# nikisalli/nightmare_rl

Measured on AMD Instinct MI355X. Metric: env-steps/sec at N parallel Nightmare-v3 envs, 1/2/4/8 MI355X, higher is better.
Workload: dtype f32; 1 GPU; 4096 Nightmare-v3 envs per GPU, random-action rollout U(-1,1)^18, full step(): 2 x 8 ms substeps (18-DoF dynamics + floor contact, PGS x3 + noslip x4) + obs/reward/termination/reset; envs_per_gpu=4096, decimation=2

## Files before the change

include/nightmare_hip.h:

```cpp
#ifndef NIGHTMARE_HIP_H
#define NIGHTMARE_HIP_H
#include <stdint.h>
#ifdef __cplusplus
extern "C" {
#endif

#define NM_NUM_OBS 66
#define NM_NUM_ACTIONS 18
#define NM_NUM_REWARDS 16
#define NM_DTYPE_F32 0
#define NM_DTYPE_F64 1

typedef struct nm_env nm_env;

typedef struct {
  int32_t decimation;
  double p_gain;
  double action_scale;
  double default_pos[3];
  double clip_actions;
  double clip_observations;
  double obs_lin_vel, obs_ang_vel, obs_dof_pos, obs_dof_vel;
  double episode_length_s;
  double resampling_time;
// ... 43 lines not shown

int nm_set_observation_noise(nm_env* env, const double* noise_scale_vec_host);
int nm_set_noise_uniforms(nm_env* env, const double* u_host);
int nm_set_push(nm_env* env, int32_t interval_steps, double max_vel_xy, uint64_t start_step);
int nm_get_push(nm_env* env, int32_t* interval_steps, double* max_vel_xy, uint64_t* step);
int nm_set_reset_noise(nm_env* env, const double* ranges10_host, const uint32_t* counts_host);
int nm_get_reset_noise(nm_env* env, int32_t* on, double* ranges10, uint32_t* counts_host);
int nm_reset_noise_offsets(const double* ranges10, uint64_t seed, int64_t global_env, uint32_t k, int32_t dtype, double* out43);
int nm_set_env_params(nm_env* env, const void* mu_dev, const void* p_gain_dev, const void* kv_dev, void* stream);
int nm_get_env_params(nm_env* env, void* mu_dev, void* p_gain_dev, void* kv_dev, void* stream);
int nm_draw_env_params(nm_env* env, const double lo[3], const double hi[3], void* stream);
int nm_set_body_params(nm_env* env, const void* rows_dev, void* stream);
int nm_get_body_params(nm_env* env, void* out_dev, void* stream);
int nm_draw_payload(nm_env* env, const double lo[4], const double hi[4], void* out_dev, void* stream);
int nm_set_action_latency(nm_env* env, const int32_t* substeps_dev, void* stream);
int nm_get_action_latency(nm_env* env, int32_t* out_dev, void* stream);
int nm_draw_action_latency(nm_env* env, int32_t lo, int32_t hi, void* stream);
int nm_set_action_history(nm_env* env, const float* hist_dev, void* stream);
int nm_get_action_history(nm_env* env, float* out_dev, void* stream);
int nm_set_gravity(nm_env* env, const void* rows_dev, void* stream);
int nm_get_gravity(nm_env* env, void* out_dev, void* stream);
int nm_draw_gravity(nm_env* env, const double lo[5], const double hi[5], void* out_dev, void* stream);
int nm_set_servo(nm_env* env, const void* rows_dev, void* stream);
int nm_get_servo(nm_env* env, void* out_dev, void* stream);
int nm_draw_servo(nm_env* env, const double lo[2], const double hi[2], void* stream);
int nm_get_servo_state(nm_env* env, double* limited);
int nm_set_servo_state(nm_env* env, const double* limited);
int nm_set_state_record(nm_env* env, int32_t env_index);
int nm_get_state_record(nm_env* env, double* qpos, double* qvel, int32_t* bad_state_resets);
int nm_get_state_log(nm_env* env, int32_t first_step, int32_t count, double* rows_host);
int nm_get_state_log_dones(nm_env* env, int32_t first_step, int32_t count, unsigned char* dones_host);

int nm_profile(nm_env* env, int32_t enable, double* sum_ms, int64_t* count);

typedef enum {
  NM_ACT_ELU = 0,
  NM_ACT_SELU = 1,
  NM_ACT_RELU = 2,
  NM_ACT_LRELU = 3,
  NM_ACT_TANH = 4,
  NM_ACT_SIGMOID = 5
} nm_activation;
#define NM_NUM_ACTIVATIONS 6

typedef struct nm_policy nm_policy;
int nm_policy_create(const int32_t* dims, int32_t n_layers, int32_t device, nm_policy** out);
int nm_policy_create_act(const int32_t* dims, int32_t n_layers, int32_t activation, int32_t device, nm_policy** out);
int nm_policy_destroy(nm_policy* h);
int nm_policy_load(nm_policy* h, const float* const* weights_dev, const float* const* bias_dev, void* stream);
int nm_policy_forward(nm_policy* h, const float* obs_dev, int32_t num_envs, float* out_dev, void* stream);

int nm_gae(const float* rewards_dev, const float* values_dev, const unsigned char* dones_dev, const float* last_values_dev,
           int32_t T, int32_t N, float gamma, float lam, float* returns_dev, void* stream);
int nm_gae_advantages(const float* rewards_dev, const float* values_dev, const unsigned char* dones_dev, const float* last_values_dev, int32_t T, int32_t N,
                      float gamma, float lam, float* returns_dev, float* advantages_dev, float* scratch_dev, int32_t normalize, void* stream);

int nm_ppo_sample(const float* net_out_dev, const float* std_dev, const float* obs_dev, int32_t N, int32_t A, int32_t n_obs, uint64_t seed,
                  const int64_t* iter_dev, int32_t step, float* actions_dev, float* logp_dev, float* values_dev, float* mu_dev, float* sigma_dev,
                  float* obs_store_dev, void* stream);
int nm_ppo_record(const float* rew_dev, const int64_t* done_dev, const float* time_outs_dev, const float* values_dev, float gamma, int32_t N,
                  float* rewards_store_dev, unsigned char* dones_store_dev, float* cur_ret_dev, float* cur_len_dev, float* fin3_dev,
                  const float* ep_stats_dev, const int32_t* ep_idx_dev, int32_t n_ep, float* ep_acc_dev, void* stream);

typedef struct nm_ppo nm_ppo;
int nm_ppo_create(const int32_t* actor_dims, const int32_t* critic_dims, int32_t n_layers, int32_t device, nm_ppo** out);
int nm_ppo_create_act(const int32_t* actor_dims, const int32_t* critic_dims, int32_t n_layers, int32_t activation, int32_t device, nm_ppo** out);
// ... 121 lines not shown
```

nightmare_rl_amd/_lib.py:

```python
import ctypes as C
import os

HERE = os.path.dirname(os.path.abspath(__file__))
LIB_PATH = os.environ.get("NM_HIP_LIB") or os.path.join(HERE, "csrc", "libnightmare_hip.so")
NUM_OBS, NUM_ACTIONS, NUM_REWARDS = 66, 18, 16
DTYPE_F32, DTYPE_F64 = 0, 1
ACTIVATIONS = {"elu": 0, "selu": 1, "relu": 2, "crelu": 2, "lrelu": 3, "tanh": 4, "sigmoid": 5}


def activation_code(name):
    try:
        return ACTIVATIONS[name]
    except (KeyError, TypeError):
        raise ValueError(f"activation {name!r} has no kernel (known: {sorted(ACTIVATIONS)})") from None


EXPORTS = ["nm_default_config", "nm_reward_name", "nm_last_error", "nm_create", "nm_destroy", "nm_num_envs", "nm_dtype", "nm_reset",
           "nm_step", "nm_step_physics", "nm_get_state", "nm_set_state", "nm_get_buffers", "nm_set_buffers",
           "nm_set_command_uniforms", "nm_get_feet_state", "nm_set_feet_state", "nm_get_counters", "nm_set_debug_buffer", "nm_set_return_accumulator", "nm_invalidate_time_outs", "nm_rollout", "nm_rollout_act", "nm_rollout_supported", "nm_policy_create", "nm_policy_destroy", "nm_policy_load", "nm_policy_forward", "nm_profile", "nm_gae", "nm_gae_advantages", "nm_ppo_sample", "nm_ppo_record", "nm_ppo_create", "nm_ppo_destroy", "nm_ppo_num_params", "nm_ppo_sync_params", "nm_ppo_minibatch", "nm_ppo_minibatch_rows", "nm_ppo_set_storage_rows", "nm_ppo_step_is_fused", "nm_ppo_debug_break_barrier", "nm_ppo_permutation", "nm_ppo_copy_grad", "nm_ppo_set_grad_buffer", "nm_ppo_get_state", "nm_ppo_snapshot_state", "nm_ppo_has_fast_path", "nm_ppo_act", "nm_ppo_record_act",
           "nm_policy_create_act", "nm_ppo_create_act", "nm_rollout_supported_act", "nm_rollout_ex", "nm_rollout_act_ex",
           "nm_set_observation_noise", "nm_set_noise_uniforms", "nm_set_state_record", "nm_get_state_record",
           "nm_get_state_log", "nm_get_state_log_dones", "nm_play", "nm_play_supported",
           "nm_nik_create", "nm_nik_destroy", "nm_nik_reset", "nm_nik_set_gait", "nm_nik_update", "nm_nik_get_state",
           "nm_step_tape", "nm_nik_tape", "nm_set_push", "nm_get_push",
           "nm_set_env_params", "nm_get_env_params", "nm_draw_env_params",
           "nm_set_body_params", "nm_get_body_params", "nm_draw_payload",
           "nm_set_action_latency", "nm_get_action_latency", "nm_draw_action_latency", "nm_set_action_history", "nm_get_action_history",
           "nm_set_reset_noise", "nm_get_reset_noise", "nm_reset_noise_offsets",
           "nm_set_gravity", "nm_get_gravity", "nm_draw_gravity",
           "nm_set_servo", "nm_get_servo", "nm_draw_servo", "nm_get_servo_state", "nm_set_servo_state"]


class NmConfig(C.Structure):
    _fields_ = [("decimation", C.c_int32), ("p_gain", C.c_double), ("action_scale", C.c_double), ("default_pos", C.c_double * 3),
                ("clip_actions", C.c_double), ("clip_observations", C.c_double),
                ("obs_lin_vel", C.c_double), ("obs_ang_vel", C.c_double), ("obs_dof_pos", C.c_double), ("obs_dof_vel", C.c_double),
                ("episode_length_s", C.c_double), ("resampling_time", C.c_double), ("max_lin_vel_x", C.c_double), ("max_ang_vel", C.c_double),
                ("termination_contact_force", C.c_double), ("tracking_sigma", C.c_double), ("reward_scales", C.c_double * NUM_REWARDS),
                ("tibia_contact_mode", C.c_int32), ("tibia_max_contact_force", C.c_double), ("body_contact_mode", C.c_int32),
                ("body_max_contact_force", C.c_double), ("base_height_target", C.c_double), ("max_contact_force", C.c_double)]


class NmRolloutArgs(C.Structure):
    _fields_ = [("steps", C.c_int32), ("params_flat_dev", C.c_void_p), ("seed", C.c_uint64), ("iter_dev", C.c_void_p),
                ("obs0_dev", C.c_void_p), ("obs_final_dev", C.c_void_p), ("episode_length_dev", C.c_void_p),
                ("rew_dev", C.c_void_p), ("done_dev", C.c_void_p), ("time_outs_dev", C.c_void_p), ("ep_stats_dev", C.c_void_p), ("bootstrap_time_outs", C.c_int32),
                ("s_obs", C.c_void_p), ("s_actions", C.c_void_p), ("s_logp", C.c_void_p), ("s_values", C.c_void_p), ("s_mu", C.c_void_p),
                ("s_sigma", C.c_void_p), ("s_rewards", C.c_void_p), ("s_dones", C.c_void_p), ("gamma", C.c_float),
                ("cur_ret", C.c_void_p), ("cur_len", C.c_void_p), ("fin3", C.c_void_p),
                ("ep_idx_dev", C.c_void_p), ("n_ep", C.c_int32), ("ep_acc_dev", C.c_void_p), ("last_values_dev", C.c_void_p)]


class NmPlayArgs(C.Structure):
    _fields_ = [("steps", C.c_int32), ("deterministic", C.c_int32), ("params_flat_dev", C.c_void_p), ("seed", C.c_uint64), ("iter_dev", C.c_void_p),
                ("step0", C.c_uint64), ("obs0_dev", C.c_void_p), ("obs_dev", C.c_void_p), ("actions_dev", C.c_void_p), ("episode_length_dev", C.c_void_p),
                ("rew_dev", C.c_void_p), ("done_dev", C.c_void_p), ("time_outs_dev", C.c_void_p), ("ep_stats_dev", C.c_void_p),
                ("cur_ret", C.c_void_p), ("cur_len", C.c_void_p), ("fin3", C.c_void_p), ("ret_sum", C.c_void_p), ("ret_cnt", C.c_void_p),
                ("ep_idx_dev", C.c_void_p), ("n_ep", C.c_int32), ("ep_acc_dev", C.c_void_p)]


class NmTapeArgs(C.Structure):
    _fields_ = [("steps", C.c_int32), ("actions_dev", C.c_void_p), ("obs_dev", C.c_void_p), ("episode_length_dev", C.c_void_p),
                ("rew_dev", C.c_void_p), ("done_dev", C.c_void_p), ("time_outs_dev", C.c_void_p), ("ep_stats_dev", C.c_void_p),
# ... 94 lines not shown
    if hasattr(L, "nm_step_tape"):
        L.nm_step_tape.argtypes = [vp, C.POINTER(NmTapeArgs), vp]
    if hasattr(L, "nm_set_push"):
        L.nm_set_push.argtypes = [vp, C.c_int32, C.c_double, C.c_uint64]
        L.nm_get_push.argtypes = [vp, C.POINTER(C.c_int32), C.POINTER(C.c_double), C.POINTER(C.c_uint64)]
    if hasattr(L, "nm_set_env_params"):
        L.nm_set_env_params.argtypes = [vp, vp, vp, vp, vp]
        L.nm_get_env_params.argtypes = [vp, vp, vp, vp, vp]
        L.nm_draw_env_params.argtypes = [vp, C.POINTER(C.c_double * 3), C.POINTER(C.c_double * 3), vp]
    if hasattr(L, "nm_set_body_params"):
        L.nm_set_body_params.argtypes = [vp, vp, vp]
        L.nm_get_body_params.argtypes = [vp, vp, vp]
        L.nm_draw_payload.argtypes = [vp, C.POINTER(C.c_double * 4), C.POINTER(C.c_double * 4), vp, vp]
    if hasattr(L, "nm_set_action_latency"):
        L.nm_set_action_latency.argtypes = [vp, vp, vp]
        L.nm_get_action_latency.argtypes = [vp, vp, vp]
        L.nm_draw_action_latency.argtypes = [vp, C.c_int32, C.c_int32, vp]
        L.nm_set_action_history.argtypes = [vp, vp, vp]
        L.nm_get_action_history.argtypes = [vp, vp, vp]
    if hasattr(L, "nm_set_reset_noise"):
        L.nm_set_reset_noise.argtypes = [vp, C.POINTER(C.c_double * 10), vp]
        L.nm_get_reset_noise.argtypes = [vp, C.POINTER(C.c_int32), C.POINTER(C.c_double * 10), vp]
        L.nm_reset_noise_offsets.argtypes = [C.POINTER(C.c_double * 10), C.c_uint64, C.c_int64, C.c_uint32, C.c_int32, C.POINTER(C.c_double * 43)]
    if hasattr(L, "nm_set_gravity"):
        L.nm_set_gravity.argtypes = [vp, vp, vp]
        L.nm_get_gravity.argtypes = [vp, vp, vp]
        L.nm_draw_gravity.argtypes = [vp, C.POINTER(C.c_double * 5), C.POINTER(C.c_double * 5), vp, vp]
    if hasattr(L, "nm_set_servo"):
        L.nm_set_servo.argtypes = [vp, vp, vp]
        L.nm_get_servo.argtypes = [vp, vp, vp]
        L.nm_draw_servo.argtypes = [vp, C.POINTER(C.c_double * 2), C.POINTER(C.c_double * 2), vp]
        L.nm_get_servo_state.argtypes = [vp, vp]
        L.nm_set_servo_state.argtypes = [vp, vp]
    if not full:
        return L
    L.nm_gae.argtypes = [vp, vp, vp, vp, C.c_int32, C.c_int32, C.c_float, C.c_float, vp, vp]
    L.nm_gae_advantages.argtypes = [vp, vp, vp, vp, C.c_int32, C.c_int32, C.c_float, C.c_float, vp, vp, vp, C.c_int32, vp]
    L.nm_ppo_sample.argtypes = [vp, vp, vp, C.c_int32, C.c_int32, C.c_int32, C.c_uint64, vp, C.c_int32, vp, vp, vp, vp, vp, vp, vp]
    L.nm_ppo_record.argtypes = [vp, vp, vp, vp, C.c_float, C.c_int32, vp, vp, vp, vp, vp, vp, vp, C.c_int32, vp, vp]
    L.nm_ppo_create.argtypes = [vp, vp, C.c_int32, C.c_int32, C.POINTER(vp)]
    L.nm_ppo_create_act.argtypes = [vp, vp, C.c_int32, C.c_int32, C.c_int32, C.POINTER(vp)]
    L.nm_ppo_destroy.argtypes = [vp]
    L.nm_ppo_num_params.argtypes = [vp]
    L.nm_ppo_sync_params.argtypes = [vp, vp, C.c_float, C.c_int64, vp]
    L.nm_ppo_minibatch.argtypes = [vp] * 12 + [C.c_int32, C.c_int32, C.c_float, C.c_float, C.c_float, C.c_int32, C.c_float, C.c_int32, C.c_float,
                                               C.c_float, C.c_float, C.c_float, C.c_int32, C.c_float, vp]
    L.nm_ppo_minibatch_rows.argtypes = [vp] * 13 + [C.c_int32, C.c_int32, C.c_float, C.c_float, C.c_float, C.c_int32, C.c_float, C.c_int32, C.c_float,
                                                    C.c_float, C.c_float, C.c_float, C.c_int32, C.c_float, vp]
    L.nm_ppo_permutation.argtypes = [vp, C.c_int32, C.c_uint64, C.c_uint64, vp]
    L.nm_ppo_copy_grad.argtypes = [vp, vp, C.c_int32, vp]
    L.nm_ppo_set_grad_buffer.argtypes = [vp, vp]
    L.nm_ppo_has_fast_path.argtypes = [vp]
    L.nm_ppo_act.argtypes = [vp, vp, vp, C.c_int32, C.c_uint64, vp, C.c_int32, vp, vp, vp, vp, vp, vp, vp]
    L.nm_ppo_record_act.argtypes = [vp, vp, vp, vp, vp, C.c_float, vp, vp, vp, vp, vp, vp, vp, C.c_int32, vp,
                                    vp, vp, C.c_int32, C.c_uint64, vp, C.c_int32, vp, vp, vp, vp, vp, vp, vp]
    L.nm_ppo_get_state.argtypes = [vp, vp, C.c_int32, vp]
    L.nm_ppo_set_storage_rows.argtypes = [vp, C.c_int64]
    L.nm_ppo_step_is_fused.argtypes = [vp]
    L.nm_ppo_step_is_fused.restype = C.c_int32
    L.nm_ppo_debug_break_barrier.argtypes = [vp, vp]
    L.nm_ppo_snapshot_state.argtypes = [vp, vp, C.c_int32, vp]
    L.nm_policy_create.argtypes = [vp, C.c_int32, C.c_int32, C.POINTER(vp)]
    L.nm_policy_create_act.argtypes = [vp, C.c_int32, C.c_int32, C.c_int32, C.POINTER(vp)]
    L.nm_policy_destroy.argtypes = [vp]
    L.nm_policy_load.argtypes = [vp, vp, vp, vp]
    L.nm_policy_forward.argtypes = [vp, vp, C.c_int32, vp, vp]
# ... 21 lines not shown
```

nightmare_rl_amd/csrc/nm_core.h:

```cpp
#pragma once
#include <type_traits>
#include <stddef.h>

#include "simt.h"

#ifdef NM_MEASURE
#define NM_ABLATE(mask) (mask)
#else
#define NM_ABLATE(mask) 0
#endif
namespace nm {
using namespace simt;

constexpr int kNQ = 25, kNV = 24, kNU = 18, kNLEG = 6, kNCOL = 7, kNSENS = 13, kNOBS = 66, kNREW = 16;
constexpr int kLinkN = 25;
constexpr int kLegN = 3 * kLinkN;
constexpr int kBaseN = 10;
constexpr int kColN = 24;
constexpr int kMaxCon = 16;
constexpr int kMaxRow = 4 * kMaxCon;
constexpr int kMaxConBig = 44;
constexpr int kBigSlots = (4 * kMaxConBig + NM_WAVE - 1) / NM_WAVE;
constexpr int kJRow = 16;
enum { R_ACTION_RATE, R_ANG_VEL_XY, R_BASE_HEIGHT, R_BODY_CONTACT, R_DEFAULT_POS, R_DOF_ACC, R_DOF_VEL, R_FEET_AIR_TIME, R_FEET_CONTACT,
// ... 96 lines not shown
  const VR d = Tt - Lo;
  return sel(vabs(d) <= rate, Tt, sel(d < VR(0), Lo - rate, Lo + rate));
}
constexpr int kDbgN = 256;

template <class Src> struct ArgSrc { static constexpr bool kScalarBase = false; };
template <class real> NM_FN const Args<real>& launch_args(const Args<real>& a) { return a; }
template <class real> NM_FN const Args<real>& launch_args(const Args<real>* a) { return *a; }
#ifndef NM_EMUL
typedef const __attribute__((address_space(4))) char* kernarg_ptr;
template <class real, int OFS> struct KernArgs { kernarg_ptr seg; };
template <class real, int OFS> struct ArgSrc<KernArgs<real, OFS>> { static constexpr bool kScalarBase = true; };
template <class real, int OFS> NM_FN const Args<real>& launch_args(const KernArgs<real, OFS>& k) {
  kernarg_ptr p = k.seg;
  asm volatile("" : "+s"(p));
  return *(const Args<real>*)(const __attribute__((address_space(4))) Args<real>*)(p + OFS);
}
template <class real, int OFS> NM_FN void launch_args_touch(const KernArgs<real, OFS>& k) {
  kernarg_ptr p = k.seg;
  asm volatile("" : "+s"(p));
  int x = 0;
#pragma unroll
  for (int o = 0; o < OFS + (int)sizeof(Args<real>); o += 64) x |= *(const __attribute__((address_space(4))) int*)(p + o);
  asm volatile("" ::"s"(x));
}
template <class real> NM_FN const Args<real>* scalar_src(const Args<real>* a) { return a; }
template <class real, int OFS> NM_FN KernArgs<real, OFS> scalar_src(const KernArgs<real, OFS>& k) {
  const uint64_t u = (uint64_t)k.seg;
  const uint32_t lo = (uint32_t)__builtin_amdgcn_readfirstlane((int)(uint32_t)u), hi = (uint32_t)__builtin_amdgcn_readfirstlane((int)(uint32_t)(u >> 32));
  return KernArgs<real, OFS>{(kernarg_ptr)(((uint64_t)hi << 32) | lo)};
}
#endif

template <class real> struct Sh {
  real qpos[kNQ];
  real envp[kEnvPS];
  real qvel[24], warm[24], ctrl[20];
  real Rb[9], wv[6];
  real anc[kNU * 3], axs[kNU * 3];
  real colR[kNCOL * 9], colp[kNCOL * 3];
  real Minv[kNLEG * 6], W[kNLEG * 18], Lb[15], Dbi[6];
  real MinvH[kNLEG * 6], WH[kNLEG * 18], LbH[15], DbiH[6];
  real qas[24], qfs[24], qfc[24];
  real vv[24];
  real sens[16], cvb[6];
  real bh[2];
  real mbb[36], sc[36];
  real legtmp[kNLEG * 66];
  NM_FN real* cpos() { return legtmp; }
  NM_FN real* cnrm() { return legtmp + 3 * kMaxConBig; }
  NM_FN real* cdist() { return legtmp + 6 * kMaxConBig; }
  NM_FN int* cleg() { return reinterpret_cast<int*>(legtmp + 7 * kMaxConBig); }
  NM_FN int* cleg1() { return reinterpret_cast<int*>(legtmp + 8 * kMaxConBig); }
  real efc_f[kMaxRow];
#ifdef NM_DEBUG_SOLVER
  real dbg_b[kMaxRow], dbg_a[kMaxRow], dbg_f0[kMaxRow];
#endif
  int ncon, nwarn, it_pgs, it_noslip, anypair;
  int nhop;
  int ntog;
  real eact[kNU], epact[kNU], epdv[kNU];
  real ecmd[4], eepsum[kNREW];
  int eplen_lo, eplen_hi;
  unsigned ectr;
  int cstart[8], ccnt[8];
  real sink[NM_WAVE];
// ... 212 lines not shown

#if defined(NM_STAMPS) && !defined(NM_EMUL)
__device__ unsigned long long g_stamps[16];
NM_FN void nm_stamp(int k) {
  __shared__ unsigned long long tl, acc[16];
#ifdef NM_STAMPS_B
  asm volatile("s_waitcnt vmcnt(0) lgkmcnt(0)" ::: "memory");
#endif
  unsigned long long n = __builtin_amdgcn_s_memtime();
  if (NM_TID == 0) {
    if (k < 0) for (int i = 0; i < 16; i++) acc[i] = 0;
    else acc[k] += n - tl;
    if (k == 10) for (int i = 0; i < 16; i++) atomicAdd(&g_stamps[i], acc[i]);
    tl = n;
  }
}
#else
NM_FN void nm_stamp(int) {}
#endif
#ifdef NM_STAMPS_B
#define NM_ESTAMP(k)
#define NM_BSTAMP(k) nm_stamp(k)
#else
#define NM_ESTAMP(k) nm_stamp(k)
#define NM_BSTAMP(k)
#endif

constexpr int kLinkTmp = 22;

template <class real> NM_FN V<real> legsum(const V<real>& x, const VB& isleg) {
  return gsum8(sel(isleg, x, V<real>(real(0))));
}

template <int EP, class real, int G> NM_FN void stage_smooth(ShW<real, G>& w, const Model<real>& M, bool last) {
  typedef V<real> vr;
  real* lds = reinterpret_cast<real*>(&w.e[0]);
  static_assert((G & (G - 1)) == 0 && 2 * G <= 8, "lane groups: G envs x 2 factorisations");
  const V<int> lane0 = opaque_lane();
  const V<int> sub = lane0 & 7, grp = lane0 >> 3;
  const V<int> leg = vmin(sub, V<int>(5)), eo = (grp & (G - 1)) * (int)(sizeof(Sh<real>) / sizeof(real));
  const VB pass1 = (grp & G) != 0;
  const VB isleg = sub < V<int>(6);
#define LDG(field, i) ldsv(lds, eo + (NM_OFS(field) + (i)))
  const V<int> bo = (grp & (G - 1)) * kBodyP + (int)(sizeof(ShW<real, G>) / sizeof(real));
#define LDB(i) ldsv(lds, bo + (i))
  const VB st_all = VB(true), st_leg = VB(true);
#define STG(field, i, val) stsv(lds, eo + (NM_OFS(field) + (i)), val, st_all)
#define LDL(field, idx) ldsv(lds, eo + (idx) + NM_OFS(field))
#define STL(field, idx, val) stsv(lds, eo + (idx) + NM_OFS(field), val, st_leg)
  const V<int> slot = leg * (3 * kLinkTmp);

  vr Rb[9];
  {
    vr qw = LDG(qpos, 3), qx = LDG(qpos, 4), qy = LDG(qpos, 5), qz = LDG(qpos, 6);
    {
      const vr in_ = vrcp(vsqrt(qw * qw + qx * qx + qy * qy + qz * qz));
      qw = qw * in_; qx = qx * in_; qy = qy * in_; qz = qz * in_;
      STG(qpos, 3, qw); STG(qpos, 4, qx); STG(qpos, 5, qy); STG(qpos, 6, qz);
    }
    vr q00 = qw * qw, q01 = qw * qx, q02 = qw * qy, q03 = qw * qz, q11 = qx * qx, q12 = qx * qy, q13 = qx * qz, q22 = qy * qy,
       q23 = qy * qz, q33 = qz * qz;
    Rb[0] = q00 + q11 - q22 - q33; Rb[4] = q00 - q11 + q22 - q33; Rb[8] = q00 - q11 - q22 + q33;
    Rb[1] = real(2) * (q12 - q03); Rb[2] = real(2) * (q13 + q02); Rb[3] = real(2) * (q12 + q03);
    Rb[5] = real(2) * (q23 - q01); Rb[6] = real(2) * (q13 - q02); Rb[7] = real(2) * (q23 + q01);
  }
  vr vb[6], ab[6];
  {
// ... 31 lines not shown
    vr Rl[9];
    Rl[0] = co + oc * ax[0] * ax[0]; Rl[1] = oc * ax[0] * ax[1] - s_ * ax[2]; Rl[2] = oc * ax[0] * ax[2] + s_ * ax[1];
    Rl[3] = oc * ax[0] * ax[1] + s_ * ax[2]; Rl[4] = co + oc * ax[1] * ax[1]; Rl[5] = oc * ax[1] * ax[2] - s_ * ax[0];
    Rl[6] = oc * ax[0] * ax[2] - s_ * ax[1]; Rl[7] = oc * ax[1] * ax[2] + s_ * ax[0]; Rl[8] = co + oc * ax[2] * ax[2];
#pragma unroll
    for (int j = 0; j < 9; j++) STL(legtmp, leg * 27 + lk * 9 + j, Rl[j]);
    wave_sync();
  }
#endif
  vr mcom[3] = {vr(real(0)), vr(real(0)), vr(real(0))};
  {
    vr Rp[9], pp[3], vpar[6], apar[6];
    vr cR[9], cpos[3], cS[6], cv[6], ca[6];
#pragma unroll
    for (int k = 0; k < 9; k++) Rp[k] = Rb[k];
    pp[0] = pp[1] = pp[2] = vr(real(0));
#pragma unroll
    for (int k = 0; k < 6; k++) { vpar[k] = vb[k]; apar[k] = ab[k]; }
#pragma unroll
    for (int k = 0; k < 3; k++) {
      sched_fence();
      const V<int> cb = leg * kLegN + k * kLinkN;
      vr q = LDL(qpos, leg * 3 + (7 + k)), qd = LDL(qvel, leg * 3 + (6 + k));
      vr pos[3], t3[3], aw[3], R[9];
      {
        vr bpos[3] = {ldsv(M.legc, cb), ldsv(M.legc, cb + 1), ldsv(M.legc, cb + 2)};
        matvec3(t3, Rp, bpos);
        pos[0] = pp[0] + t3[0]; pos[1] = pp[1] + t3[1]; pos[2] = pp[2] + t3[2];
      }
      {
        vr ax[3] = {ldsv(M.legc, cb + 12), ldsv(M.legc, cb + 13), ldsv(M.legc, cb + 14)};
        vr R0[9];
        {
          if (uniform(M.link_rot_id[k])) {
#pragma unroll
            for (int j = 0; j < 9; j++) R0[j] = Rp[j];
          } else {
            vr bR[9];
#pragma unroll
            for (int j = 0; j < 9; j++) bR[j] = ldsv(M.legc, cb + 3 + j);
            matmul3(R0, Rp, bR);
          }
        }
        matvec3(aw, R0, ax);
        vr Rl[9];
#ifndef NM_NO_ROLE_ROT
#pragma unroll
        for (int j = 0; j < 9; j++) Rl[j] = LDL(legtmp, leg * 27 + (k * 9 + j));
        (void)q;
#else
        vr s, co;
        vsincos(q, &s, &co);
        vr oc = vr(real(1)) - co;
        Rl[0] = co + oc * ax[0] * ax[0]; Rl[1] = oc * ax[0] * ax[1] - s * ax[2]; Rl[2] = oc * ax[0] * ax[2] + s * ax[1];
        Rl[3] = oc * ax[0] * ax[1] + s * ax[2]; Rl[4] = co + oc * ax[1] * ax[1]; Rl[5] = oc * ax[1] * ax[2] - s * ax[0];
        Rl[6] = oc * ax[0] * ax[2] - s * ax[1]; Rl[7] = oc * ax[1] * ax[2] + s * ax[0]; Rl[8] = co + oc * ax[2] * ax[2];
#endif
        matmul3(R, R0, Rl);
      }
#pragma unroll
      for (int j = 0; j < 3; j++) {
        STL(anc, leg * 9 + (3 * k + j), pos[j]);
        STL(axs, leg * 9 + (3 * k + j), aw[j]);
      }
      if (k == 2) {
#pragma unroll
        for (int j = 0; j < 9; j++) STL(colR, (leg + 1) * 9 + j, R[j]);
// ... 619 lines not shown
  wmaxfirst(best, &sv, &si);
  if (popc64(ballot(best == vr(sv))) == 1) return rdlane(ibest, si);
  wargmax(best, ibest, &sv, &si);
  return si;
}
template <class real> NM_FN real hull_tie_tol() { return sizeof(real) == 8 ? real(1e-13) : real(4e-7); }
constexpr int kMaxHop = 3;
template <class real> constexpr real kObbSlack() { return real(1e-5); }

constexpr int kSelfLane = 63;
constexpr int kSlackScale = 1 << 20;
constexpr int kBatchLane0 = kSelfLane + 1 - kNCOL;
template <class real> NM_FN void hull_ring(const Model<real>& M, int gv, V<int>& nbg, V<real>* v) {
  const V<int> lane = lane_id();
  const VB nbl = lane < M.maxnbr;
  V<real> o[4];
  gld4(M.hullnv, (sel(nbl, lane, V<int>(M.maxnbr)) + gv * (M.maxnbr + 1)) * 4, o);
  v[0] = o[0]; v[1] = o[1]; v[2] = o[2];
  nbg = to_int(o[3]);
}
template <class real> struct Rings {
  V<int> nb[kNCOL];
  V<real> vv[kNCOL][3];
  int cur[kNCOL];
};
template <class real> NM_FN void collide_rings(const Sh<real>& sh, const Model<real>& M, Rings<real>& r) {
#pragma unroll
  for (int g = 0; g < kNCOL; g++) {
    const int vadr = (int)M.colc[kColN * g + 6];
    r.cur[g] = uniform(sh.hcache[g]);
    hull_ring(M, vadr + r.cur[g], r.nb[g], r.vv[g]);
  }
}
template <class real> NM_FN void stage_collide(Sh<real>& sh, const Model<real>& M, int* dropped, Rings<real>& rg, bool pairs = true) {
  typedef V<real> vr;
  const V<int> lane = lane_id();
  const real bz = sh.qpos[2];
  const VB nbl = lane < M.maxnbr;
  V<int>* nb = rg.nb;
  vr (*vv)[3] = rg.vv;
  int* cur = rg.cur;
  real pz[kNCOL], ldv[kNCOL][3], sv[kNCOL];
  bool near[kNCOL];
  vr val[kNCOL];
#pragma unroll
  for (int g = 0; g < kNCOL; g++) {
    const real* R = sh.colR + 9 * g;
    const real* cc = M.colc + kColN * g;
    pz[g] = sh.colp[3 * g + 2] + bz;
    const real cz = R[6] * cc[0] + R[7] * cc[1] + R[8] * cc[2] + pz[g];
    near[g] = !(cz - cc[3] > real(0));
    ldv[g][0] = -R[6]; ldv[g][1] = -R[7]; ldv[g][2] = -R[8];
    val[g] = ldv[g][0] * vv[g][0] + ldv[g][1] * vv[g][1] + ldv[g][2] * vv[g][2];
    sv[g] = rdlane(val[g], kSelfLane);
  }
  NM_BSTAMP(11);
#pragma unroll
  for (int g = 0; g < kNCOL; g++) {
    const real tol = hull_tie_tol<real>();
    if (near[g] && wany(nbl & (nb[g] >= 0) & (val[g] >= vr(sv[g] - tol)))) {
      {
        const real* cc = M.colc + kColN * g;
        real top = ldv[g][0] * cc[8] + ldv[g][1] * cc[9] + ldv[g][2] * cc[10];
#pragma unroll
        for (int a = 0; a < 3; a++) top += cc[20 + a] * vabs(ldv[g][0] * cc[11 + 3 * a] + ldv[g][1] * cc[12 + 3 * a] + ldv[g][2] * cc[13 + 3 * a]);
        if (uniform(pz[g] - top > kObbSlack<real>())) { near[g] = false; continue; }
      }
// ... 10 lines not shown
        si = rdlane(nb[g], lbest);
        NM_BSTAMP(12);
        hull_ring(M, vadr + si, nb[g], vv[g]);
        val[g] = ld[0] * vv[g][0] + ld[1] * vv[g][1] + ld[2] * vv[g][2];
        sv[g] = rdlane(val[g], kSelfLane);
        NM_BSTAMP(14);
        sh.nhop += 1;
      }
      if (full) {
        NM_BSTAMP(12);
        const int held = si;
        si = support_exhaustive(M, ld, nvert, vadr);
        sh.hcache[7] += 1;
#ifdef NM_MEASURE
        sh.nhop += g == 0 ? 1000 : 100000;
#endif
        if (si != held) {
          hull_ring(M, vadr + si, nb[g], vv[g]);
          val[g] = ld[0] * vv[g][0] + ld[1] * vv[g][1] + ld[2] * vv[g][2];
          sv[g] = rdlane(val[g], kSelfLane);
        }
        NM_BSTAMP(15);
      }
      if (si != cur[g]) sh.hcache[g] = si;
    }
  }
  NM_BSTAMP(12);
  int total = 0;
  unsigned hitbits = 0;
#pragma unroll
  for (int g = 0; g < kNCOL; g++) hitbits |= (uniform(near[g] && pz[g] - sv[g] < real(0)) ? 1u : 0u) << g;
  const int nhit = popc64(hitbits);
  bool batch = false;
  if (nhit >= M.collide_batch_min) {
    const uint64_t hitm = (uint64_t)hitbits << kBatchLane0;
    vr X[3] = {vv[kNCOL - 1][0], vv[kNCOL - 1][1], vv[kNCOL - 1][2]}, svl = val[kNCOL - 1];
    V<int> slackl = nb[kNCOL - 1];
    V<int> lb = lane;
#pragma unroll
    for (int g = kNCOL - 2; g >= 0; g--) {
      order_after(lb, X[0]);
      const VB mg = lb == kBatchLane0 + g;
      X[0] = sel(mg, vv[g][0], X[0]); X[1] = sel(mg, vv[g][1], X[1]); X[2] = sel(mg, vv[g][2], X[2]);
      svl = sel(mg, val[g], svl);
      slackl = sel(mg, nb[g], slackl);
    }
    const VB ml = lane >= kBatchLane0;
    const V<int> gl = sel(ml, lane - kBatchLane0, V<int>(0));
    const vr pzl = ldsv(sh.colp, gl * 3 + 2) + bz;
    const vr distl = pzl - svl;
    const VB wr = in_mask(hitm);
    const VB lone = distl * real(-0.5 * kSlackScale) < to_real<real>(slackl);
    if (!wany(wr & !lone)) {
      vr Rl[9], pl[2], pnt[3];
#pragma unroll
      for (int j = 0; j < 9; j++) Rl[j] = ldsv(sh.colR, gl * 9 + j);
#pragma unroll
      for (int j = 0; j < 2; j++) pl[j] = ldsv(sh.colp, gl * 3 + j);
      matvec3_fma(pnt, Rl, X);
      pnt[0] = pnt[0] + pl[0]; pnt[1] = pnt[1] + pl[1]; pnt[2] = pnt[2] + ldsv(sh.colp, gl * 3 + 2);
      const V<int> slot = lane_rank(hitm);
      const V<int> sl = sel(wr, slot, V<int>(0));
      stsv(sh.cpos(), sl * 3, pnt[0], wr);
      stsv(sh.cpos(), sl * 3 + 1, pnt[1], wr);
      stsv(sh.cpos(), sl * 3 + 2, pnt[2] - real(0.5) * distl, wr);
      stsv(sh.cdist(), sl, distl, wr);
      stsv(sh.cleg(), sl, gl - 1, wr);
// ... 70 lines not shown
      f(std::integral_constant<int, C>{});
      for_contacts<C + 1, N>(ncon, f);
    }
  }
}
template <class F> NM_FN void sfor4(F&& f) {
  f(std::integral_constant<int, 0>{}); f(std::integral_constant<int, 1>{}); f(std::integral_constant<int, 2>{}); f(std::integral_constant<int, 3>{});
}
template <int NP, int P = 0, class F> NM_FN void sfor_pairs(int ncon, F&& f) {
  if constexpr (P < NP) {
    if (P / 2 < ncon) {
      f(std::integral_constant<int, P>{});
      f(std::integral_constant<int, P + 1>{});
      sfor_pairs<NP, P + 2>(ncon, f);
    }
  }
}
template <class X> NM_FN void pgs_row_prepare(const X& Rr, const X& f, const X& ARinv, X& k0, X& k1, X& nf) {
  k0 = -ARinv;
  k1 = (Rr * f) * k0;
  nf = -f;
}
template <class X> NM_FN X pgs_row_delta(const X& g, const X& k0, const X& k1, const X& nf) { return vmax(vfma(g, k0, k1), nf); }
template <class X> NM_FN X pgs_row_cost(const X& dl, const X& hA, const X& g, const X& Rr, const X& f) { return dl * vfma(hA, dl, vfma(Rr, f, g)); }
template <class real, class X, class B> NM_FN void noslip_pair_prepare(const X& f, const X& fp, const B& small, X& lo, X& hi) {
  const X mean = real(0.5) * (fp - f);
  lo = sel(small, mean, -f);
  hi = sel(small, mean, fp);
}
template <class X> NM_FN X noslip_pair_delta(const X& dg, const X& invK1, const X& lo, const X& hi) { return vmin(vmax(-dg * invK1, lo), hi); }
template <class X> NM_FN X noslip_pair_cost(const X& d, const X& hK1, const X& dg) { return d * vfma(hK1, d, dg); }
template <class real, class X> NM_FN auto noslip_pair_bad(const X& change) { return change > X(real(1e-10)); }

template <class real, bool PAIR, int EP> NM_FN void stage_constraint_body(Sh<real>& sh, real* jrow, const Model<real>& M, bool last, bool nosweep, BodyRef<EP, real> br) {
  typedef V<real> vr;
  const V<int> lane = lane_id();
  const int ncon = uniform(sh.ncon), nefc = 4 * ncon;
  if (nefc == 0) {
#pragma unroll
    for (int j = 0; j < 24; j++) sh.qfc[j] = real(0);
    if (last)
#pragma unroll
      for (int j = 0; j < kNSENS; j++) sh.sens[j] = real(0);
    wave_sync();
    return;
  }
  const VB act = lane < nefc;
  const V<int> c = sel(act, lane >> 2, V<int>(0));
  const V<int> tk = (lane >> 1) & 1, sg = lane & 1;
  vr cp[3] = {ldsv(sh.cpos(), c * 3), ldsv(sh.cpos(), c * 3 + 1), ldsv(sh.cpos(), c * 3 + 2)};
  vr dist = ldsv(sh.cdist(), c);
  V<int> L = ldsv(sh.cleg(), c);
  const VB onleg = L >= 0;
  const V<int> Lc = vmax(L, V<int>(0));
  constexpr bool anypair = PAIR;
  V<int> L1 = V<int>(-1);
  if (anypair) L1 = ldsv(sh.cleg1(), c);
  const VB onleg1 = L1 >= 0;
  const V<int> Lc1 = vmax(L1, V<int>(0));
  const V<int> q4 = lane & 3;
  vr smu = sel(sg == 0, vr(env_mu<EP>(sh, M)), vr(-env_mu<EP>(sh, M)));
  vr nrm[3] = {vr(real(0)), vr(real(0)), vr(real(1))};
  vr e[3] = {sel(q4 == 2, vr(real(-1)), vr(real(0))), sel(q4 == 1, vr(real(1)), vr(real(0))), sel((q4 == 0) | (q4 == 3), vr(real(1)), vr(real(0)))};
  if (anypair) {
    nrm[0] = ldsv(sh.cnrm(), c * 3); nrm[1] = ldsv(sh.cnrm(), c * 3 + 1); nrm[2] = ldsv(sh.cnrm(), c * 3 + 2);
    VB usey = (nrm[1] < vr(real(0.5))) & (nrm[1] > vr(real(-0.5)));
    vr y0[3] = {vr(real(0)), sel(usey, vr(real(1)), vr(real(0))), sel(usey, vr(real(0)), vr(real(1)))};
// ... 53 lines not shown
    for (int k = 0; k < 3; k++) uF[j] = uF[j] - ldsv(sh.W, Lc * 18 + (6 * k + j)) * Fl[k];
  }
  if (anypair) {
#pragma unroll
    for (int j = 0; j < 6; j++)
#pragma unroll
      for (int k = 0; k < 3; k++) uF[j] = uF[j] - ldsv(sh.W, Lc1 * 18 + (6 * k + j)) * Fm[k];
  }
#pragma unroll
  for (int j = 0; j < 6; j++) stsv(jrow, lane * kJRow + j, uF[j], lane < kMaxRow);
#pragma unroll
  for (int k = 0; k < 3; k++) stsv(jrow, lane * kJRow + (6 + k), Fl[k], lane < kMaxRow);
  if (anypair) {
#pragma unroll
    for (int k = 0; k < 3; k++) stsv(jrow, lane * kJRow + (10 + k), Fm[k], lane < kMaxRow);
  }
  vr Jb[6], Jl[3], Jm[3] = {vr(real(0)), vr(real(0)), vr(real(0))};
#pragma unroll
  for (int j = 0; j < 6; j++) Jb[j] = quad<0x00>(Fb[j]) + smu * quad<0xA5>(Fb[j]);
#pragma unroll
  for (int k = 0; k < 3; k++) Jl[k] = quad<0x00>(Fl[k]) + smu * quad<0xA5>(Fl[k]);
  if (anypair) {
#pragma unroll
    for (int k = 0; k < 3; k++) Jm[k] = quad<0x00>(Fm[k]) + smu * quad<0xA5>(Fm[k]);
  }
  vr u[6];
#pragma unroll
  for (int j = 0; j < 6; j++) u[j] = quad<0x00>(uF[j]) + smu * quad<0xA5>(uF[j]);

  vr imp;
  {
    vr x = vabs(dist) * vrcp(M.si_width);
    vr ylo, yhi;
    if (M.si_power == real(2)) {
      vr omx = vmax(vr(real(1)) - x, vr(real(0)));
      ylo = (x * x) * vrcp(M.si_mid);
      yhi = vr(real(1)) - (omx * omx) * vrcp(real(1) - M.si_mid);
    } else {
      ylo = vpow(x, vr(M.si_power)) / vpow(vr(M.si_mid), vr(M.si_power - real(1)));
      yhi = vr(real(1)) - vpow(vmax(vr(real(1)) - x, vr(real(0))), vr(M.si_power)) / vpow(vr(real(1) - M.si_mid), vr(M.si_power - real(1)));
    }
    vr y = sel(x <= vr(M.si_mid), ylo, yhi);
    imp = M.si_d0 + y * (M.si_dmax - M.si_d0);
    imp = sel(x >= vr(real(1)), vr(M.si_dmax), imp);
    imp = sel(x <= vr(real(0)), vr(M.si_d0), imp);
  }
  vr invw = body_invw(br, M, Lc + sel(onleg, V<int>(1), V<int>(0)));
  if (anypair) invw = invw + sel(onleg1, body_invw(br, M, Lc1 + 1), vr(real(0)));
  vr Rr = vmax((vr(real(1)) - imp) * (invw + env_mu<EP>(sh, M) * env_mu<EP>(sh, M) * invw) * vrcp(imp), vr(real(1e-15))) * (real(2) * env_mu<EP>(sh, M) * env_mu<EP>(sh, M));
  vr Dd = vrcp(Rr);
  vr vel = vr(real(0)), jas = vr(real(0)), jaw = vr(real(0));
#pragma unroll
  for (int j = 0; j < 6; j++) {
    vel += Jb[j] * sh.qvel[j]; jas += Jb[j] * sh.qas[j]; jaw += Jb[j] * sh.warm[j];
  }
#pragma unroll
  for (int k = 0; k < 3; k++) {
    V<int> di = Lc * 3 + (6 + k);
    vel += Jl[k] * ldsv(sh.qvel, di); jas += Jl[k] * ldsv(sh.qas, di); jaw += Jl[k] * ldsv(sh.warm, di);
  }
  if (anypair) {
#pragma unroll
    for (int k = 0; k < 3; k++) {
      V<int> di = Lc1 * 3 + (6 + k);
      vel += Jm[k] * ldsv(sh.qvel, di); jas += Jm[k] * ldsv(sh.qas, di); jaw += Jm[k] * ldsv(sh.warm, di);
    }
  }
  vr aref = -M.solref_B * vel - M.solref_K * imp * dist;
  vr bb = jas - aref;

// ... 185 lines not shown
    const V<int> lg = sel(on, (lane * 13) >> 6, V<int>(0)), qq = lane - lg * 5;
    const V<int> c0 = ldsv(sh.cstart, lg + 1), cn = ldsv(sh.ccnt, lg + 1);
    vr acc = vr(real(0));
#pragma unroll
    for (int k = 0; k < 4; k++) {
      VB in = on & (cn > k);
      acc = acc + sel(in, ldsv(jrow, sel(in, (c0 + k) * 8 + qq, V<int>(0))), vr(real(0)));
    }
    stsv(sh.qfc, 6 + lg * 3 + qq, acc, on & (qq < 3));
    if (last) {
      stsv(sh.sens, lg, acc, on & (qq == 3));
      stsv(sh.sens, lg + 6, acc, on & (qq == 4));
      sh.sens[12] = wsum<real>(sel(act & ((lane & 3) == 0) & (L < 0), tn, vr(real(0))));
    }
  } else {
#pragma unroll
    for (int l = 0; l < 6; l++)
#pragma unroll
      for (int k = 0; k < 3; k++) sh.qfc[6 + 3 * l + k] = wsum<real>(sel(L == l, Jl[k] * f, vr(real(0))) + sel(L1 == l, Jm[k] * f, vr(real(0))));
    if (last) {
      VB head = act & ((lane & 3) == 0) & (nf > vr(real(0)));
#pragma unroll
      for (int l = 0; l < 6; l++) {
        VB onl = (L == l) | (L1 == l);
        sh.sens[l] = wsum<real>(sel(head & onl, nf, vr(real(0))));
        sh.sens[6 + l] = wsum<real>(sel(head & (((L == l) & hit) | ((L1 == l) & hit1)), nf, vr(real(0))));
      }
      sh.sens[12] = wsum<real>(sel(head & (L < 0), nf, vr(real(0))));
    }
  }
  wave_sync();
}

template <class real, int EP> NM_COLD void stage_constraint_pairs(Sh<real>& sh, real* jrow, const Model<real>& M, bool last, bool nosweep, BodyRef<EP, real> br) {
  stage_constraint_body<real, true, EP>(sh, jrow, M, last, nosweep, br);
}

constexpr int kMaxCon2 = 8, kMaxRow2 = 4 * kMaxCon2;
#ifdef NM_EMUL
inline long& nm_emul_together() { static long n = 0; return n; }
#endif
template <int EP, class real> NM_FN void stage_constraint2(ShW<real, 2>& w, const Model<real>& M, bool last, bool nosweep) {
  typedef V<real> vr;
  constexpr int kSR = (int)(sizeof(Sh<real>) / sizeof(real)), kSI = (int)(sizeof(Sh<real>) / sizeof(int));
  const V<int> lane = lane_id();
  const V<int> h = lane >> 5, hl = lane & 31;
  const VB h1 = h != 0;
  real* rbw = reinterpret_cast<real*>(&w.e[0]);
  int* ibw = reinterpret_cast<int*>(&w.e[0]);
  const real* rb = rbw;
  const int* ib = ibw;
  real* jrow = w.jrow;
  const V<int> ho = h * kSR, hoi = h * kSI, jh = h * (kMaxRow2 * kJRow);
  const int oLeg = NM_OFS(legtmp);
  const int oCleg = (int)((offsetof(Sh<real>, legtmp) + 7 * kMaxConBig * sizeof(real)) / sizeof(int));
#define SHR(field, idx) ldsv(rb, ho + ((idx) + NM_OFS(field)))
#define SHI(field, idx) ldsv(ib, hoi + ((idx) + NM_IOFS(field)))
  const int n0 = uniform(w.e[0].ncon), n1 = uniform(w.e[1].ncon), nmax = vmax(n0, n1);
  const V<int> nconv = sel(h1, V<int>(n1), V<int>(n0)), nefc = nconv * 4;
  const VB act = hl < nefc;
  const V<int> c = sel(act, hl >> 2, V<int>(0));
  const V<int> sg = hl & 1;
  vr cp[3] = {ldsv(rb, ho + (c * 3 + oLeg)), ldsv(rb, ho + (c * 3 + (oLeg + 1))), ldsv(rb, ho + (c * 3 + (oLeg + 2)))};
  vr dist = ldsv(rb, ho + (c + (oLeg + 6 * kMaxConBig)));
  V<int> L = ldsv(ib, hoi + (c + oCleg));
  {
    const VB any = nconv > 0;
    cp[0] = sel(any, cp[0], vr(real(0))); cp[1] = sel(any, cp[1], vr(real(0))); cp[2] = sel(any, cp[2], vr(real(0)));
    dist = sel(any, dist, vr(real(0)));
    L = sel(any, L, V<int>(-1));
  }
  const VB onleg = L >= 0;
  const V<int> Lc = vmax(L, V<int>(0));
  const V<int> q4 = hl & 3;
  auto mu2 = [&]() -> vr { if constexpr (EP != 0) return SHR(envp, V<int>(EP_MU)); else return vr(M.mu); };
// ... 24 lines not shown
      }
      cross3(mm, rel, e);
      Fl[k] = sel(onleg, dot3<vr>(a, mm), vr(real(0)));
    }
  }
#pragma unroll
  for (int j = 0; j < 6; j++) Fb[j] = sel(act, Fb[j], vr(real(0)));
#pragma unroll
  for (int k = 0; k < 3; k++) Fl[k] = sel(act, Fl[k], vr(real(0)));
  vr uF[6];
#pragma unroll
  for (int j = 0; j < 6; j++) {
    uF[j] = Fb[j];
#pragma unroll
    for (int k = 0; k < 3; k++) uF[j] = uF[j] - SHR(W, Lc * 18 + (6 * k + j)) * Fl[k];
  }
#pragma unroll
  for (int j = 0; j < 6; j++) stsv(jrow, lane * kJRow + j, uF[j], VB(true));
#pragma unroll
  for (int k = 0; k < 3; k++) stsv(jrow, lane * kJRow + (6 + k), Fl[k], VB(true));
  vr Jb[6], Jl[3];
#pragma unroll
  for (int j = 0; j < 6; j++) Jb[j] = quad<0x00>(Fb[j]) + smu * quad<0xA5>(Fb[j]);
#pragma unroll
  for (int k = 0; k < 3; k++) Jl[k] = quad<0x00>(Fl[k]) + smu * quad<0xA5>(Fl[k]);
  vr u[6];
#pragma unroll
  for (int j = 0; j < 6; j++) u[j] = quad<0x00>(uF[j]) + smu * quad<0xA5>(uF[j]);

  vr imp;
  {
    vr x = vabs(dist) * vrcp(M.si_width);
    vr ylo, yhi;
    if (M.si_power == real(2)) {
      vr omx = vmax(vr(real(1)) - x, vr(real(0)));
      ylo = (x * x) * vrcp(M.si_mid);
      yhi = vr(real(1)) - (omx * omx) * vrcp(real(1) - M.si_mid);
    } else {
      ylo = vpow(x, vr(M.si_power)) / vpow(vr(M.si_mid), vr(M.si_power - real(1)));
      yhi = vr(real(1)) - vpow(vmax(vr(real(1)) - x, vr(real(0))), vr(M.si_power)) / vpow(vr(real(1) - M.si_mid), vr(M.si_power - real(1)));
    }
    vr y = sel(x <= vr(M.si_mid), ylo, yhi);
    imp = M.si_d0 + y * (M.si_dmax - M.si_d0);
    imp = sel(x >= vr(real(1)), vr(M.si_dmax), imp);
    imp = sel(x <= vr(real(0)), vr(M.si_d0), imp);
  }
  vr invw;
  if constexpr (EP >= 2) invw = ldsv(bp2, hb + (Lc + sel(onleg, V<int>(1), V<int>(0)) + BP_INVW));
  else invw = ldsv(M.colc, (Lc + sel(onleg, V<int>(1), V<int>(0))) * kColN + 4);
  vr Rr = vmax((vr(real(1)) - imp) * (invw + MU2 * MU2 * invw) * vrcp(imp), vr(real(1e-15))) * (real(2) * MU2 * MU2);
  vr Dd = vrcp(Rr);
  vr vel = vr(real(0)), jas = vr(real(0)), jaw = vr(real(0));
#pragma unroll
  for (int j = 0; j < 6; j++) {
    vel += Jb[j] * SHR(qvel, V<int>(j)); jas += Jb[j] * SHR(qas, V<int>(j)); jaw += Jb[j] * SHR(warm, V<int>(j));
  }
#pragma unroll
  for (int k = 0; k < 3; k++) {
    V<int> di = Lc * 3 + (6 + k);
    vel += Jl[k] * SHR(qvel, di); jas += Jl[k] * SHR(qas, di); jaw += Jl[k] * SHR(warm, di);
  }
  vr aref = -M.solref_B * vel - M.solref_K * imp * dist;
  vr bb = jas - aref;

  vr t[3], xb[6];
  {
    vr Mi[6];
#pragma unroll
    for (int j = 0; j < 6; j++) Mi[j] = SHR(Minv, Lc * 6 + j);
    ldl3_solve(t, Mi, Jl);
// ... 529 lines not shown
        vr dif[3] = {cp[0] - ft[0], cp[1] - ft[1], cp[2] - ft[2]};
        vr b2 = sgn * (nrm[0] * dif[0] + nrm[1] * dif[1] + nrm[2] * dif[2]);
        vr cc = dif[0] * dif[0] + dif[1] * dif[1] + dif[2] * dif[2] - fr * fr;
        vr det = b2 * b2 - cc;
        vr sq = vsqrt(vmax(det, vr(real(0))));
        return !(det < vr(real(1e-15))) & (((-b2 - sq) >= vr(real(0))) | ((-b2 + sq) >= vr(real(0))));
      };
      const VB hit = foot_hit(vmax(r.L[k], V<int>(0)), real(-1)), hit1 = foot_hit(vmax(r.L1[k], V<int>(0)), real(1));
      const VB head = r.act[k] & ((lane & 3) == 0) & (nf > vr(real(0)));
#pragma unroll
      for (int l = 0; l < kNLEG; l++) {
        s_all[l] += sel(head & ((r.L[k] == l) | (r.L1[k] == l)), nf, vr(real(0)));
        s_foot[l] += sel(head & (((r.L[k] == l) & hit) | ((r.L1[k] == l) & hit1)), nf, vr(real(0)));
      }
      s_base += sel(head & (r.L[k] < 0), nf, vr(real(0)));
    }
#pragma unroll
    for (int l = 0; l < kNLEG; l++) { sh.sens[l] = wsum<real>(s_all[l]); sh.sens[6 + l] = wsum<real>(s_foot[l]); }
    sh.sens[12] = wsum<real>(s_base);
  }
  wave_sync();
}
template <class real> NM_COLD void floor_frames(Sh<real>& sh) {
  const V<int> lane = lane_id();
  const int nfloor = uniform(sh.cstart[7]);
  const VB on = lane < nfloor;
  const V<int> c = sel(on, lane, V<int>(0));
  stsv(sh.cleg1(), c, V<int>(-1), on);
  stsv(sh.cnrm(), c * 3, V<real>(real(0)), on);
  stsv(sh.cnrm(), c * 3 + 1, V<real>(real(0)), on);
  stsv(sh.cnrm(), c * 3 + 2, V<real>(real(1)), on);
  wave_sync();
}
template <class real, int EP> NM_FN void stage_constraint(Sh<real>& sh, real* jrow, const Model<real>& M, bool last, bool nosweep, BodyRef<EP, real> br) {
  if (uniform(sh.ncon) > kMaxCon) { floor_frames(sh); stage_constraint_big<real, EP>(sh, M, last, nosweep, br); }
  else if (uniform(sh.anypair) != 0) { floor_frames(sh); stage_constraint_pairs<real, EP>(sh, jrow, M, last, nosweep, br); }
  else stage_constraint_body<real, false, EP>(sh, jrow, M, last, nosweep, br);
}

template <class real, int G, int EP = 0> NM_FN void stage_integrate(ShW<real, G>& w, const Model<real>& M) {
  typedef V<real> vr;
  real* lds = reinterpret_cast<real*>(&w.e[0]);
  const V<int> lane0 = opaque_lane();
  const V<int> sub = lane0 & 7, grp = lane0 >> 3;
  const V<int> leg = vmin(sub, V<int>(5)), eo = (grp & (G - 1)) * (int)(sizeof(Sh<real>) / sizeof(real));
  const VB pass1 = (grp & G) != 0;
  const VB isleg = sub < V<int>(6);
#define LDG(field, i) ldsv(lds, eo + (NM_OFS(field) + (i)))
#define LDL(field, idx) ldsv(lds, eo + (idx) + NM_OFS(field))
  constexpr int kFacH = NM_OFS(MinvH) - NM_OFS(Minv);
  static_assert(NM_OFS(WH) - NM_OFS(W) == kFacH && NM_OFS(LbH) - NM_OFS(Lb) == kFacH && NM_OFS(DbiH) - NM_OFS(Dbi) == kFacH, "factor blocks");
  static_assert(sizeof(Sh<real>::mbb) / sizeof(real) >= 24 && sizeof(Sh<real>::sc) / sizeof(real) >= 28 && sizeof(Sh<real>::vv) / sizeof(real) >= 24, "junk rows");
  const V<int> eoF = eo + sel(pass1, V<int>(kFacH), V<int>(0));
  vr xl[3], xb[6];
  {
    vr y[3], t[3], Mi[6];
#pragma unroll
    for (int k = 0; k < 3; k++) y[k] = LDL(qfc, leg * 3 + (6 + k)) + sel(pass1, LDL(qfs, leg * 3 + (6 + k)), vr(real(0)));
#pragma unroll
    for (int j = 0; j < 6; j++) Mi[j] = ldsv(lds, eoF + leg * 6 + (NM_OFS(Minv) + j));
    ldl3_solve(t, Mi, y);
#pragma unroll
    for (int j = 0; j < 6; j++) {
      vr wy = ldsv(lds, eoF + leg * 18 + (NM_OFS(W) + j)) * y[0] + ldsv(lds, eoF + leg * 18 + (NM_OFS(W) + 6 + j)) * y[1] +
              ldsv(lds, eoF + leg * 18 + (NM_OFS(W) + 12 + j)) * y[2];
      xb[j] = LDG(qfc, j) - legsum<real>(wy, isleg) + sel(pass1, LDG(qfs, j), vr(real(0)));
    }
    {
      vr L[15], Di[6];
#pragma unroll
// ... 92 lines not shown
      stsv(sh.warm, lane, sel(lane == 2, vr(-M.grav), vr(real(0))), lane < kNV);
      }
      stsv(sh.ctrl, lane, real(0), lane < kNU);
      wave_sync();
    }
  }
#undef LDG
#undef LDL
}

template <class real> NM_FN void reset_data(Sh<real>& sh, const Model<real>& M) {
  const V<int> lane = opaque_lane();
  stsv(sh.qpos, lane, ldsv(M.qpos0, sel(lane < kNQ, lane, V<int>(0))), lane < kNQ);
  stsv(sh.qvel, lane, real(0), lane < kNV);
  stsv(sh.warm, lane, real(0), lane < kNV);
  stsv(sh.ctrl, lane, real(0), lane < kNU);
  wave_sync();
}

#ifndef NM_PRIO
#define NM_PRIO 3
#endif
#if !defined(NM_EMUL)
NM_FN void nm_set_priority(int load) {
  if (load >= NM_PRIO + 4) __builtin_amdgcn_s_setprio(3);
  else if (load >= NM_PRIO + 2) __builtin_amdgcn_s_setprio(2);
  else if (load >= NM_PRIO) __builtin_amdgcn_s_setprio(1);
  else __builtin_amdgcn_s_setprio(0);
}
#else
inline void nm_set_priority(int) {}
#endif

template <int EP, class real, int G> NM_FN void substep(ShW<real, G>& w, const Model<real>& M, bool last, int* dropped, int ablate) {
  const V<int> lane = opaque_lane();
  if constexpr (G == 2) {
    constexpr int kSR = (int)(sizeof(Sh<real>) / sizeof(real));
    real* rbw = reinterpret_cast<real*>(&w.e[0]);
    const V<int> hl = lane & 31, ho = (lane >> 5) * kSR;
    {
      const VB bad = (visbad(ldsv(rbw, ho + (sel(hl < kNQ, hl, V<int>(0)) + NM_OFS(qpos)))) & (hl < kNQ)) |
                     (visbad(ldsv(rbw, ho + (sel(hl < kNV, hl, V<int>(0)) + NM_OFS(qvel)))) & (hl < kNV));
      const uint64_t bm = ballot(bad);
      if (bm) {
#pragma unroll
        for (int e = 0; e < 2; e++)
          if ((bm >> (32 * e)) & 0xffffffffull) { w.e[e].nwarn += 1; reset_data(w.e[e], M); }
      }
    }
  } else {
    for (int e = 0; e < G; e++) {
      Sh<real>& sh = w.e[e];
      {
        VB bad = (visbad(ldsv(sh.qpos, sel(lane < kNQ, lane, V<int>(0)))) & (lane < kNQ)) |
                 (visbad(ldsv(sh.qvel, sel(lane < kNV, lane, V<int>(0)))) & (lane < kNV));
        if (wany(bad)) { sh.nwarn += 1; reset_data(sh, M); }
      }
    }
  }
  wave_sync();
  nm_stamp(1);
  if (!(ablate & 8)) stage_smooth<EP>(w, M, last);
  nm_stamp(2);
  for (int e = 0; e < G; e++) {
    Sh<real>& sh = w.e[e];
    if (!(ablate & 1)) { Rings<real> rg; collide_rings(sh, M, rg); stage_collide(sh, M, dropped, rg, G != 2 && !(ablate & 16)); }
    else { sh.ncon = 0; sh.anypair = 0; wave_sync(); }
  }
  if constexpr (G == 2) {
    if (!(ablate & 1) && !(ablate & 16)) stage_collide_pairs2(w, M, dropped);
  }
  for (int e = 0; e < G; e++)
    if (ablate & 4) { w.e[e].ncon = 0; w.e[e].anypair = 0; wave_sync(); }
  bool together = false;
  if constexpr (G == 2) {
    const int n0 = uniform(w.e[0].ncon), n1 = uniform(w.e[1].ncon);
    nm_set_priority(n0 + n1);
    together = n0 + n1 >= 1 && n0 <= kMaxCon2 && n1 <= kMaxCon2 && uniform(w.e[0].anypair) == 0 && uniform(w.e[1].anypair) == 0 && !(ablate & 32);
    if (!last) w.e[1].ntog = n0 * 64 + n1;
    if (together) {
#ifdef NM_EMUL
      nm_emul_together() += 1;
#endif
      w.e[0].ntog += 1;
      stage_constraint2<EP>(w, M, last, (ablate & 2) != 0);
      nm_stamp(8);
    }
  }
  if (!together)
    for (int e = 0; e < G; e++) {
      BodyRef<EP, real> br;
      if constexpr (EP >= 2) br = BodyRef<EP, real>(body_rows(w) + e * kBodyP);
      stage_constraint<real, EP>(w.e[e], w.jrow, M, last, (ablate & 2) != 0, br);
      nm_stamp(8);
    }
  if constexpr (EP >= 4) stage_integrate<real, G, EP>(w, M);
  else
  stage_integrate(w, M);
  nm_stamp(9);
}


template <int EP, class real> NM_FN void env_load(Sh<real>& sh, const Model<real>& M, const Args<real>& A, int env, real* bp = nullptr,
                                                real* late = nullptr, int* rsw = nullptr, bool live = true, real* gp = nullptr) {
  typedef V<real> vr;
  const V<int> lane = opaque_lane();
  const VB l18 = lane < kNU;
  const V<int> l18c = sel(l18, lane, V<int>(0));
  const vr q_in = gldv(A.qpos, sel(lane < kNQ, lane, V<int>(0)) + env * kNQ);
  const vr v_in = gldv(A.qvel, sel(lane < kNV, lane, V<int>(0)) + env * kNV);
  const vr w_in = gldv(A.qwarm, sel(lane < kNV, lane, V<int>(0)) + env * kNV);
  const V<int> hc_in = gldv(A.hullcache, sel(lane < 8, lane, V<int>(0)) + env * 8);
  const V<float> a_in = gldv(A.actions, l18c + env * kNU);
  vr envp_in = vr(real(0));
  if constexpr (EP != 0) envp_in = gldv(A.envp, sel(lane < kEnvP, lane, V<int>(0)) + env * kEnvP);
  vr body_in = vr(real(0));
  if constexpr (EP >= 2) body_in = gldv(A.envp, sel(lane < kBodyP, lane, V<int>(0)) + (A.N * kEnvP + env * kBodyP));
  vr grav_in = vr(real(0));
  if constexpr (EP >= 4) grav_in = gldv(grav_rows_of(A), sel(lane < kGravP, lane, V<int>(0)) + env * kGravP);
  vr cmd_in = vr(real(0)), eps_in = vr(real(0)), prev_act = vr(real(0)), prev_dofvel = vr(real(0)), dofpos_old = vr(real(0));
  int64_t ep = 0;
  uint32_t ctr_in = 0;
  int dl = 0;
  V<float> h0 = V<float>(0.0f), h1 = V<float>(0.0f), h2 = V<float>(0.0f);
  if constexpr (EP >= 3)
    if (!A.physics_only) {
// ... 331 lines not shown
#else
      if (m) gst1(A.obs, (size_t)env * kNOBS + idx, (float)cx);
#endif
    };
    put(o, lane, lane < 12);
    put((dofpos - defp) * M.obs_dofpos, lane + 12, l18);
    put(dofvel * M.obs_dofvel, lane + 30, l18);
    put(act, lane + 48, l18);
  }
  NM_ESTAMP(15);
  gstv(A.dofpos, lane + env * kNU, dofpos, l18);
  gstv(A.dofvel, lane + env * kNU, dofvel, l18);
  gstv(A.act, lane + env * kNU, act, l18);
  {
    vr cv = sel(lane == 0, vr(cmd[0]), sel(lane == 1, vr(cmd[1]), vr(cmd[2])));
    gstv(A.cmd, lane + env * 3, cv, lane < 3);
  }
#ifdef NM_EMUL
  const bool lane0 = true;
#else
  const bool lane0 = NM_TID == 0;
#endif
  if (lane0) {
    gst1(A.eplen, env, eplen);
    gst1(A.rngctr, env, ctr);
    gst1(A.rew, env, (float)rew);
    if (A.ret_acc) gadd1(A.ret_acc, env, (float)rew);
    gst1(A.done, env, (int64_t)(reset ? 1 : 0));
    gst1(A.timeout_now, env, time_out ? 1.0f : 0.0f);
  }
}

struct NoMid { NM_FN void operator()() const {} NM_FN void operator()(int) const {} };
template <int EP, class real, class Src, class Mid> NM_FN void env_load2(ShW<real, 2>& w, const Model<real>& M, const Src& src, int wave, Mid&& mid) {
  typedef V<real> vr;
  const Args<real>& A = launch_args(src);
  constexpr bool kS = ArgSrc<Src>::kScalarBase;
  constexpr int kSR = (int)(sizeof(Sh<real>) / sizeof(real)), kSI = (int)(sizeof(Sh<real>) / sizeof(int));
  const V<int> lane = opaque_lane();
  const V<int> h = lane >> 5, hl = lane & 31;
  const V<int> env0 = h + wave * 2;
  const V<int> env = sel(env0 < V<int>(A.N), env0, V<int>(A.N - 1));
  real* rb = reinterpret_cast<real*>(&w.e[0]);
  int* ib = reinterpret_cast<int*>(&w.e[0]);
  const V<int> ho = h * kSR, hoi = h * kSI;
  const VB l18 = hl < kNU;
  const V<int> l18c = sel(l18, hl, V<int>(0));
  const vr q_in = gldx<kS>(A.qpos, sel(hl < kNQ, hl, V<int>(0)) + env * kNQ);
  const vr v_in = gldx<kS>(A.qvel, sel(hl < kNV, hl, V<int>(0)) + env * kNV);
  const vr w_in = gldx<kS>(A.qwarm, sel(hl < kNV, hl, V<int>(0)) + env * kNV);
  const V<int> hc_in = gldx<kS>(A.hullcache, sel(hl < 8, hl, V<int>(0)) + env * 8);
  const V<float> a_in = gldx<kS>(A.actions, l18c + env * kNU);
  vr envp_in = vr(real(0));
  if constexpr (EP != 0) envp_in = gldx<kS>(A.envp, sel(hl < kEnvP, hl, V<int>(0)) + env * kEnvP);
  vr body_in = vr(real(0));
  if constexpr (EP >= 2) body_in = gldx<kS>(A.envp, sel(hl < kBodyP, hl, V<int>(0)) + (env * kBodyP + A.N * kEnvP));
  vr grav_in = vr(real(0));
  if constexpr (EP >= 4) grav_in = gldx<kS>(grav_rows_of(A), sel(hl < kGravP, hl, V<int>(0)) + env * kGravP);
  vr cmd_in = vr(real(0)), eps_in = vr(real(0)), prev_act = vr(real(0)), prev_dofvel = vr(real(0)), dofpos_old = vr(real(0));
  V<int> dl = V<int>(0);
  V<float> h0 = V<float>(0.0f), h1 = V<float>(0.0f), h2 = V<float>(0.0f);
  if constexpr (EP >= 3)
    if (!A.physics_only) {
      dl = gldx<kS>(lat_delay(A), env);
      h0 = gldx<kS>(lat_hist(A), l18c + env * (kLatH * kNU));
      h1 = gldx<kS>(lat_hist(A), l18c + (env * (kLatH * kNU) + kNU));
      h2 = gldx<kS>(lat_hist(A), l18c + (env * (kLatH * kNU) + 2 * kNU));
    }
  vr servo_in = vr(real(0)), lim_in = vr(real(0));
  if constexpr (EP >= 5)
    if (!A.physics_only) {
      servo_in = gldx<kS>(servo_rows_of(A), sel(hl < kServoP, hl, V<int>(0)) + env * kServoP);
      lim_in = gldx<kS>(servo_state_of(A), l18c + env * kNU);
    }
#ifndef NM_EMUL
  int64_t ep = 0;
  uint32_t ctr_in = 0;
#endif
  if (!A.physics_only) {
    cmd_in = gldx<kS>(A.cmd, sel(hl < 3, hl, V<int>(0)) + env * 3);
    eps_in = gldx<kS>(A.epsum, sel(hl < kNREW, hl, V<int>(0)) + env * kNREW);
#ifndef NM_EMUL
    ep = gld1x<kS>(A.eplen, env);
    ctr_in = gld1x<kS>(A.rngctr, env);
#endif
    prev_act = gldx<kS>(A.act, l18c + env * kNU);
    prev_dofvel = gldx<kS>(A.dofvel, l18c + env * kNU);
    dofpos_old = gldx<kS>(A.dofpos, l18c + env * kNU);
  }
  mid();
  stsv(rb, ho + (hl + NM_OFS(qpos)), q_in, hl < kNQ);
  stsv(rb, ho + (hl + NM_OFS(qvel)), v_in, hl < kNV);
  stsv(rb, ho + (hl + NM_OFS(warm)), w_in, hl < kNV);
  stsv(ib, hoi + (hl + NM_IOFS(hcache)), sel(hl == 0, hc_in & V<int>(0xffff), hc_in), hl < 8);
  nm_set_priority((rdlane(hc_in, 0) >> 16) + (rdlane(hc_in, 32) >> 16));
  w.e[0].nwarn = 0; w.e[1].nwarn = 0;
  w.e[0].nhop = 0; w.e[1].nhop = 0;
  w.e[0].ntog = 0; w.e[1].ntog = 0;
  vr p_gain = vr(M.p_gain);
  if constexpr (EP != 0) {
    stsv(rb, ho + (hl + NM_OFS(envp)), envp_in, hl < kEnvPS);
    if constexpr (EP >= 2) stsv(body_rows(w), h * kBodyP + hl, body_in, hl < kBodyP);
    if constexpr (EP >= 4) stsv(grav_rows(w), h * kGravP + hl, grav_in, hl < kGravP);
    p_gain = sel(h != 0, vr(rdlane(envp_in, 32 + EP_PGAIN)), vr(rdlane(envp_in, EP_PGAIN)));
  }
  V<float> af = a_in * M.action_scale;
  af = vmin(vmax(af, V<float>(-M.clip_actions)), V<float>(M.clip_actions));
  vr act;
  vr defp;
  {
    V<int> m3 = hl % 3;
    defp = sel(m3 == 1, vr(M.default_pos[1]), sel(m3 == 0, vr(M.default_pos[0]), vr(M.default_pos[2])));
  }
#ifdef NM_EMUL
  for (int i = 0; i < NM_WAVE; i++) act.v[i] = (real)af.v[i];
#else
  act = (real)af;
#endif
  if (!A.physics_only) {
    stsv(rb, ho + (hl + NM_OFS(ecmd)), cmd_in, hl < 3);
    stsv(rb, ho + (hl + NM_OFS(eepsum)), eps_in, hl < kNREW);
#ifdef NM_EMUL
    for (int hh = 0; hh < 2; hh++) {
      const int e = env.v[32 * hh];
      const int64_t ep = A.eplen[e];
      w.e[hh].eplen_lo = (int)(uint32_t)(ep & 0xffffffffll);
      w.e[hh].eplen_hi = (int)(ep >> 32);
      w.e[hh].ectr = A.rngctr[e];
    }
#else
    stsv(ib, hoi + NM_IOFS(eplen_lo), (int)(uint32_t)(ep & 0xffffffffll), hl == 0);
    stsv(ib, hoi + NM_IOFS(eplen_hi), (int)(ep >> 32), hl == 0);
    stsv(ib, hoi + NM_IOFS(ectr), (int)ctr_in, hl == 0);
#endif
    if constexpr (EP >= 3) {
      const V<int> ns = V<int>(A.nsub), one = V<int>(1), zero = V<int>(0);
      const V<int> k = sel(dl >= ns, one, zero) + sel(dl >= ns + ns, one, zero) + sel(dl >= ns + ns + ns, one, zero), r = dl - k * ns;
      const V<float> fl = sel(k == zero, af, sel(k == one, h0, sel(k == V<int>(2), h1, h2)));
      const V<float> fe = sel(r > zero, sel(k == zero, h0, sel(k == one, h1, h2)), fl);
      ShWL<real, 2>& L = lat_rows(w);
      if constexpr (EP >= 5) {
        const vr rate = sel(h != 0, vr(rdlane(servo_in, 32 + SV_RATE)), vr(rdlane(servo_in, SV_RATE)));
        const vr d_gain = sel(h != 0, vr(rdlane(servo_in, 32 + SV_DGAIN)), vr(rdlane(servo_in, SV_DGAIN)));
        const vr lim = servo_limit(lim_in, vcvt<real>(fl) - defp, rate);
        const vr damp = prev_dofvel * d_gain;
        stsv(rb, ho + (hl + NM_OFS(ctrl)), (sel(r > zero, lim_in, lim) - dofpos_old) * p_gain - damp, l18);
        stsv(L.late, h * kNU + hl, (lim - dofpos_old) * p_gain - damp, l18);
        gstx<kS>(servo_state_of(A), hl + env * kNU, lim, l18 & (env0 < V<int>(A.N)));
      } else {
      stsv(rb, ho + (hl + NM_OFS(ctrl)), ((vcvt<real>(fe) - defp) - dofpos_old) * p_gain, l18);
      stsv(L.late, h * kNU + hl, ((vcvt<real>(fl) - defp) - dofpos_old) * p_gain, l18);
      }
      stsv(L.rsw, h, r, hl == zero);
      float* hist = lat_hist(A);
      const VB st = l18 & (env0 < V<int>(A.N));
      gstx<kS>(hist, hl + (env * (kLatH * kNU) + 2 * kNU), h1, st);
      gstx<kS>(hist, hl + (env * (kLatH * kNU) + kNU), h0, st);
      gstx<kS>(hist, hl + env * (kLatH * kNU), af, st);
    } else
    stsv(rb, ho + (hl + NM_OFS(ctrl)), ((act - defp) - dofpos_old) * p_gain, l18);
  } else {
    wave_sync();
    stsv(rb, ho + (hl + NM_OFS(ctrl)), ((act - defp) - ldsv(rb, ho + (l18c + (7 + NM_OFS(qpos))))) * p_gain, l18);
    if constexpr (EP >= 3) stsv(lat_rows(w).rsw, h, V<int>(0), hl == V<int>(0));
  }
  stsv(rb, ho + (hl + NM_OFS(eact)), act, l18); stsv(rb, ho + (hl + NM_OFS(epact)), prev_act, l18); stsv(rb, ho + (hl + NM_OFS(epdv)), prev_dofvel, l18);
  wave_sync();
}

template <int EP = 0, class real, class Src, class Pub> NM_FN void env_finish2(ShW<real, 2>& w, const Model<real>& M, const Src& src, int wave, int dropped, Pub&& published) {
  typedef V<real> vr;
  const Args<real>& A = launch_args(src);
  constexpr bool kS = ArgSrc<Src>::kScalarBase;
  constexpr int kSR = (int)(sizeof(Sh<real>) / sizeof(real)), kSI = (int)(sizeof(Sh<real>) / sizeof(int));
  const V<int> lane = opaque_lane();
  const V<int> h = lane >> 5, hl = lane & 31;
  const VB h1 = h != 0;
  const V<int> env = h + wave * 2;
  const VB live = env < V<int>(A.N);
  const V<int> envc = sel(live, env, V<int>(A.N - 1));
  const bool lives[2] = {wave * 2 < A.N, wave * 2 + 1 < A.N};
  const real* rb = reinterpret_cast<const real*>(&w.e[0]);
  const int* ib = reinterpret_cast<const int*>(&w.e[0]);
  const V<int> ho = h * kSR, hoi = h * kSI;
#define SHR(field, idx) ldsv(rb, ho + ((idx) + NM_OFS(field)))
#define SHI(field, idx) ldsv(ib, hoi + ((idx) + NM_IOFS(field)))
  const VB l18 = hl < kNU;
  const V<int> l18c = sel(l18, hl, V<int>(0));
  const vr act = SHR(eact, l18c), prev_act = SHR(epact, l18c), prev_dofvel = SHR(epdv, l18c);
  vr defp;
  {
    V<int> m3 = hl % 3;
    defp = sel(m3 == 1, vr(M.default_pos[1]), sel(m3 == 0, vr(M.default_pos[0]), vr(M.default_pos[2])));
  }
  const V<int> nwarn = SHI(nwarn, V<int>(0));
  {
    V<int> hc = SHI(hcache, sel(hl < 8, hl, V<int>(0)));
    hc = sel(hl == 0, hc | (SHI(ncon, V<int>(0)) << 16), hc);
    const vr q = SHR(qpos, sel(hl < kNQ, hl, V<int>(0))), v = SHR(qvel, sel(hl < kNV, hl, V<int>(0))), wq = SHR(warm, sel(hl < kNV, hl, V<int>(0)));
    gstx<kS>(A.hullcache, hl + env * 8, hc, live & (hl < 8));
    gstx<kS>(A.qpos, hl + env * kNQ, q, live & (hl < kNQ));
    gstx<kS>(A.qvel, hl + env * kNV, v, live & (hl < kNV));
    gstx<kS>(A.qwarm, hl + env * kNV, wq, live & (hl < kNV));
    if (A.rec) {
      const VB r = live & (env == V<int>(A.rec_env));
      gstx<kS>(A.rec, hl, q, r & (hl < kNQ));
      gstx<kS>(A.rec, hl + kNQ, v, r & (hl < kNV));
      gstx<kS>(A.rec, V<int>(kNQ + kNV), to_real<real>(nwarn), r & (hl == 0));
    }
  }
  if (A.dbg) {
    if (lives[0]) env_debug(w.e[0], A, wave * 2, dropped);
    if (lives[1]) env_debug(w.e[1], A, wave * 2 + 1, 0);
  }
  if (A.stat_cnt && (dropped != 0 || wany(live & (nwarn != 0)))) {
#ifdef NM_EMUL
    A.stat_cnt[1] += dropped;
    for (int hh = 0; hh < 2; hh++) if (lives[hh]) A.stat_cnt[2] += nwarn.v[32 * hh];
#else
    if (NM_TID == 0 && dropped) nm_consume(atomicAdd(A.stat_cnt + 1, dropped));
    if (hl == 0 && live && nwarn) nm_consume(atomicAdd(A.stat_cnt + 2, nwarn));
#endif
  }
  if (A.physics_only) return;
  if (NM_ABLATE(A.ablate) & 128) return;
  NM_ESTAMP(11);

  int64_t ep[2];
  uint32_t ctr[2];
#pragma unroll
  for (int hh = 0; hh < 2; hh++) {
    ep[hh] = (((int64_t)w.e[hh].eplen_hi << 32) | (int64_t)(uint32_t)w.e[hh].eplen_lo) + 1;
    ctr[hh] = w.e[hh].ectr;
  }
  vr bq[4] = {SHR(qpos, V<int>(3)), -SHR(qpos, V<int>(4)), -SHR(qpos, V<int>(5)), -SHR(qpos, V<int>(6))};
  auto rot = [&](vr* r, const vr* v) {
    vr tx = real(2) * (bq[2] * v[2] - bq[3] * v[1]), ty = real(2) * (bq[3] * v[0] - bq[1] * v[2]), tz = real(2) * (bq[1] * v[1] - bq[2] * v[0]);
    r[0] = v[0] + bq[0] * tx + (bq[2] * tz - bq[3] * ty);
    r[1] = v[1] + bq[0] * ty + (bq[3] * tx - bq[1] * tz);
    r[2] = v[2] + bq[0] * tz + (bq[1] * ty - bq[2] * tx);
  };
  vr blv[3], bav[3], pg[3];
  {
    vr lin[3] = {SHR(cvb, V<int>(3)), SHR(cvb, V<int>(4)), SHR(cvb, V<int>(5))}, ang[3] = {SHR(cvb, V<int>(0)), SHR(cvb, V<int>(1)), SHR(cvb, V<int>(2))};
    vr gv[3] = {vr(real(0)), vr(real(0)), vr(-M.grav)};
    if constexpr (EP >= 4) {
      const real* gr = grav_rows(w);
      const V<int> go = h * kGravP + GP_VEC;
      gv[0] = ldsv(gr, go); gv[1] = ldsv(gr, go + 1); gv[2] = ldsv(gr, go + 2);
    }
    rot(blv, lin); rot(bav, ang); rot(pg, gv);
  }
  vr dofpos = SHR(qpos, l18c + 7), dofvel = SHR(qvel, l18c + 6);
  vr tib[6], feet[6], body = SHR(sens, V<int>(12));
#pragma unroll
  for (int l = 0; l < 6; l++) {
    feet[l] = SHR(sens, V<int>(6 + l));
    tib[l] = sel(feet[l] == vr(real(0)), SHR(sens, V<int>(l)), vr(real(0)));
  }
  vr cmd[3] = {SHR(ecmd, V<int>(0)), SHR(ecmd, V<int>(1)), SHR(ecmd, V<int>(2))};
  auto resample = [&](int hh, int which) {
    const int e = wave * 2 + hh;
    real ux, uy;
    if (A.cmd_u) { ux = gld1(A.cmd_u, (size_t)(e * 4 + 2 * which)); uy = gld1(A.cmd_u, (size_t)(e * 4 + 2 * which + 1)); }
    else {
      ux = (real)rand_u24_bits(A.seed, (uint64_t)(A.env_offset + e), ctr[hh]) * real(1.0 / 16777216.0);
      uy = (real)rand_u24_bits(A.seed, (uint64_t)(A.env_offset + e), ctr[hh] + 1) * real(1.0 / 16777216.0);
      ctr[hh] += 2;
    }
    real c0 = ux * real(2) * M.max_lin_x - M.max_lin_x, c1 = real(0), c2 = uy * real(2) * M.max_ang - M.max_ang;
    real keep = vsqrt(c0 * c0 + c1 * c1) > real(0.02) ? real(1) : real(0);
    c0 = c0 * keep; c1 = c1 * keep;
    const VB mine = hh ? h1 : !h1;
    cmd[0] = sel(mine, vr(c0), cmd[0]); cmd[1] = sel(mine, vr(c1), cmd[1]); cmd[2] = sel(mine, vr(c2), cmd[2]);
  };
  bool tos[2];
#pragma unroll
  for (int hh = 0; hh < 2; hh++) {
    bool due;
    if (ep[hh] >= 0 && ep[hh] < (1 << 22)) {
      const int e32 = (int)ep[hh], R = M.resample_every;
      const int q = (int)((float)e32 / (float)R);
      const int r = e32 - q * R;
      due = r == 0 || r == R || r == -R;
    } else due = ep[hh] % M.resample_every == 0;
    if (due && lives[hh]) resample(hh, 0);
    tos[hh] = (real)ep[hh] > M.max_ep_len;
  }
  const VB time_out = (h1 & VB(tos[1])) | (!h1 & VB(tos[0]));
  VB reset = time_out;
  {
    vr fm = feet[0];
#pragma unroll
    for (int l = 1; l < 6; l++) fm = vmax(fm, feet[l]);
    reset = reset | (fm > vr(M.term_force));
    if ((M.tibia_mode == 2) | (M.body_mode == 2)) {
      vr tm = tib[0];
#pragma unroll
      for (int l = 1; l < 6; l++) tm = vmax(tm, tib[l]);
      if (M.tibia_mode == 2) reset = reset | (tm > vr(M.tibia_max));
      if (M.body_mode == 2) reset = reset | (body > vr(M.body_max));
    }
    vr nrm = vsqrt(pg[0] * pg[0] + pg[1] * pg[1] + pg[2] * pg[2]);
    if (sizeof(real) == 8) reset = reset | (vacos(-pg[2] / nrm) > vr(real(1.0471975511965976)));
    else reset = reset | ((-pg[2] / nrm) <= vr(real(0.5)));
  }
  NM_ESTAMP(12);
  vr epsum = SHR(eepsum, sel(hl < kNREW, hl, V<int>(0)));
  const VB resetL = reset & live;
  const uint64_t rmask = ballot(resetL);
  if (rmask) {
    gstx<kS>(A.qpos, hl + env * kNQ, ldsv(M.qpos0, sel(hl < kNQ, hl, V<int>(0))), resetL & (hl < kNQ));
    gstx<kS>(A.qvel, hl + env * kNV, real(0), resetL & (hl < kNV));
#pragma unroll
    for (int hh = 0; hh < 2; hh++)
      if ((rmask >> (32 * hh)) & 1) { resample(hh, 1); ep[hh] = 0; }
#ifdef NM_EMUL
    for (int hh = 0; hh < 2; hh++)
      if ((rmask >> (32 * hh)) & 1) {
        for (int k = 0; k < kNREW; k++) A.stat_sum[k] += epsum.v[32 * hh + k];
        A.stat_cnt[0] += 1;
      }
#else
    if (resetL && hl < kNREW) nm_consume(atomicAdd(A.stat_sum + hl, epsum));
    if (resetL && hl == 0) {
      nm_consume(atomicAdd(A.stat_cnt, 1));
      if (time_out && A.to_list) nm_consume(atomicExch(A.to_list + atomicAdd(A.nto, 1), env));
    }
#endif
    epsum = sel(resetL, vr(real(0)), epsum);
  }
  published(0);
  NM_ESTAMP(13);
  vr rt[kNREW];
#pragma unroll
  for (int k = 0; k < kNREW; k++) rt[k] = vr(real(0));
  {
    vr da = prev_act - act;
    rt[R_ACTION_RATE] = hsum32(sel(l18, da * da, vr(real(0)))) * M.rew_scale[R_ACTION_RATE];
    vr sumt = ((tib[0] + tib[1]) + (tib[2] + tib[3])) + (tib[4] + tib[5]);
    if ((M.tibia_mode != 1) | (M.body_mode != 1)) {
      sumt = M.tibia_mode == 1 ? sumt : vr(real(0));
      body = M.body_mode == 1 ? body : vr(real(0));
    }
    rt[R_BODY_CONTACT] = (sumt + body) * M.rew_scale[R_BODY_CONTACT];
    vr dp = dofpos - defp;
    rt[R_DEFAULT_POS] = hsum32(sel(l18, dp * dp, vr(real(0)))) * M.rew_scale[R_DEFAULT_POS];
    vr acc = (dofvel - prev_dofvel) / M.dt;
    rt[R_DOF_ACC] = hsum32(sel(l18, acc * acc, vr(real(0)))) * M.rew_scale[R_DOF_ACC];
    rt[R_ORIENTATION] = (pg[0] * pg[0] + pg[1] * pg[1]) * M.rew_scale[R_ORIENTATION];
    vr ea = (cmd[2] - bav[2]) * (cmd[2] - bav[2]);
    rt[R_TRACK_ANG] = vexp(-ea / M.sigma) * M.rew_scale[R_TRACK_ANG];
    vr el = (cmd[0] - blv[0]) * (cmd[0] - blv[0]) + (cmd[1] - blv[1]) * (cmd[1] - blv[1]);
    rt[R_TRACK_LIN] = vexp(-el / M.sigma) * M.rew_scale[R_TRACK_LIN];
    rt[R_TERMINATION] = sel(reset & !time_out, vr(M.rew_scale[R_TERMINATION]), vr(real(0)));
    if (M.rew_extra) {
      rt[R_ANG_VEL_XY] = (bav[0] * bav[0] + bav[1] * bav[1]) * M.rew_scale[R_ANG_VEL_XY];
      vr dh = SHR(bh, V<int>(0)) - M.base_h_target;
      rt[R_BASE_HEIGHT] = dh * dh * M.rew_scale[R_BASE_HEIGHT];
      rt[R_DOF_VEL] = hsum32(sel(l18, dofvel * dofvel, vr(real(0)))) * M.rew_scale[R_DOF_VEL];
      rt[R_LIN_VEL_Z] = blv[2] * blv[2] * M.rew_scale[R_LIN_VEL_Z];
      vr still = sel(vsqrt(cmd[0] * cmd[0] + cmd[1] * cmd[1]) < vr(real(0.01)), vr(real(1)), vr(real(0)));
      rt[R_STAND_STILL] = hsum32(sel(l18, vabs(dp), vr(real(0)))) * still * M.rew_scale[R_STAND_STILL];
      const VB l6 = hl < kNLEG;
      const V<int> l6c = sel(l6, hl, V<int>(0));
      const vr ff = SHR(sens, l6c + 6);
      vr over = sel(ff > vr(M.max_contact_force), ff - M.max_contact_force, vr(real(0)));
      rt[R_FEET_CONTACT] = hsum32(sel(l6, over * over, vr(real(0)))) * M.rew_scale[R_FEET_CONTACT];
      if (M.rew_scale[R_FEET_AIR_TIME] != real(0)) {
        vr air = gldx<kS>(A.feetair, l6c + envc * kNLEG);
        const V<int> fl = gldx<kS>(A.feetflags, envc);
        air = sel(reset, vr(real(0)), air);
        const VB contact = ff > vr(real(1));
        const VB filt = contact | (((fl >> l6c) & 1) != 0);
        const VB lastf = ((fl >> (l6c + kNLEG)) & 1) != 0;
        air = air + M.dt;
        air = sel(filt == lastf, air, vr(real(0)));
        const vr single = sel(air > vr(real(1)), air - real(1), vr(real(0))) + sel(air < vr(real(0.5)), real(0.5) - air, vr(real(0)));
        rt[R_FEET_AIR_TIME] = hsum32(sel(l6, single * single, vr(real(0)))) * M.rew_scale[R_FEET_AIR_TIME];
        gstx<kS>(A.feetair, l6c + env * kNLEG, air, live & l6);
        const uint64_t bc = ballot(l6 & contact), bf = ballot(l6 & filt);
        const int nf0 = (int)((bc & 63) | ((bf & 63) << kNLEG)), nf1 = (int)(((bc >> 32) & 63) | (((bf >> 32) & 63) << kNLEG));
        gstx<kS>(A.feetflags, env, sel(h1, V<int>(nf1), V<int>(nf0)), live & (hl == 0));
      }
    }
  }
  vr rew = vr(real(0));
#pragma unroll
  for (int k = 0; k < kNREW; k++) rew = rew + rt[k];
  {
    vr add = vr(real(0));
#pragma unroll
    for (int k = 0; k < kNREW; k++) add = sel(hl == k, rt[k], add);
    gstx<kS>(A.epsum, hl + env * kNREW, epsum + add, live & (hl < kNREW));
  }
  published(1);
  NM_ESTAMP(14);
  if (!(NM_ABLATE(A.ablate) & 256)) {
    vr head[12] = {blv[0] * M.obs_lin, blv[1] * M.obs_lin, blv[2] * M.obs_lin, bav[0] * M.obs_ang, bav[1] * M.obs_ang, bav[2] * M.obs_ang,
                   pg[0], pg[1], pg[2], cmd[0] * M.obs_lin, cmd[1] * M.obs_lin, cmd[2] * M.obs_ang};
    vr o = vr(real(0));
#pragma unroll
    for (int k = 0; k < 12; k++) o = sel(hl == k, head[k], o);
    auto put = [&](const vr& x0, const V<int>& idx, const VB& m0) {
      const VB m = m0 & live;
      vr x = x0;
      if (A.noise_vec) {
        auto nz = [&](int k, int e) {
          real u = A.noise_u ? gld1(A.noise_u, (size_t)e * kNOBS + k)
                             : (real)rand_u24_bits(A.seed + kNoiseKey, (uint64_t)(A.env_offset + e), (uint32_t)(A.noise_step * kNOBS + k)) * real(1.0 / 16777216.0);
          return (real(2) * u - real(1)) * gld1(A.noise_vec, (size_t)k);
        };
#ifdef NM_EMUL
        for (int i = 0; i < NM_WAVE; i++) if (m.v[i]) x.v[i] = x.v[i] + nz(idx.v[i], env.v[i]);
#else
        if (m) x = x + nz(idx, env);
#endif
      }
      vr cx = vmin(vmax(x, vr(-M.clip_obs)), vr(M.clip_obs));
#ifdef NM_EMUL
      for (int i = 0; i < NM_WAVE; i++) if (m.v[i]) A.obs[(size_t)env.v[i] * kNOBS + idx.v[i]] = (float)cx.v[i];
#else
      if constexpr (kS) { if (m) gst1x<true>(A.obs, env * kNOBS + idx, (float)cx); }
      else if (m) gst1(A.obs, (size_t)env * kNOBS + idx, (float)cx);
#endif
    };
    put(o, hl, hl < 12);
    put((dofpos - defp) * M.obs_dofpos, hl + 12, l18);
    put(dofvel * M.obs_dofvel, hl + 30, l18);
    put(act, hl + 48, l18);
  }
  NM_ESTAMP(15);
  gstx<kS>(A.dofpos, hl + env * kNU, dofpos, live & l18);
  gstx<kS>(A.dofvel, hl + env * kNU, dofvel, live & l18);
  gstx<kS>(A.act, hl + env * kNU, act, live & l18);
  {
    vr cv = sel(hl == 0, cmd[0], sel(hl == 1, cmd[1], cmd[2]));
    gstx<kS>(A.cmd, hl + env * 3, cv, live & (hl < 3));
  }
#ifdef NM_EMUL
// ... 6 lines not shown
    }
#else
  if (hl == 0 && live) {
    gst1x<kS>(A.eplen, env, h1 ? ep[1] : ep[0]);
    gst1x<kS>(A.rngctr, env, h1 ? ctr[1] : ctr[0]);
    gst1x<kS>(A.rew, env, (float)rew);
    if (A.ret_acc) gadd1x<kS>(A.ret_acc, env, (float)rew);
    gst1x<kS>(A.done, env, (int64_t)(reset ? 1 : 0));
    gst1x<kS>(A.timeout_now, env, time_out ? 1.0f : 0.0f);
  }
#endif
#undef SHR
#undef SHI
}

template <class real, int G> NM_FN void latency_switch(ShW<real, G>& w, int s) {
  ShWL<real, G>& L = lat_rows(w);
  const V<int> lane = opaque_lane();
  wave_sync();
  if constexpr (G == 2) {
    constexpr int kSR = (int)(sizeof(Sh<real>) / sizeof(real));
    real* rb = reinterpret_cast<real*>(&w.e[0]);
    const V<int> h = lane >> 5, hl = lane & 31;
    const VB on = (hl < kNU) & (ldsv(L.rsw, h) == V<int>(s));
    const V<real> cmd = ldsv(L.late, h * kNU + sel(hl < kNU, hl, V<int>(0)));
    stsv(rb, h * kSR + (hl + NM_OFS(ctrl)), cmd, on);
  } else {
    for (int e = 0; e < G; e++)
      if (uniform(L.rsw[e]) == s) stsv(w.e[e].ctrl, lane, ldsv(L.late, sel(lane < kNU, lane, V<int>(0)) + e * kNU), lane < kNU);
  }
  wave_sync();
}

template <class real, int G, int EP = 0, class Mid = NoMid, class Pub = NoMid, class Src = Args<real>>
NM_FN void wave_step(ShW<real, G>& w, const Model<real>& M, const Src& src, int wave, Mid&& mid = Mid(), Pub&& published = Pub()) {
  const Args<real>& A = launch_args(src);
  nm_stamp(-1);
  if constexpr (G == 2) {
    env_load2<EP>(w, M, src, wave, mid);
  } else {
    mid();
#pragma unroll
    for (int e = 0; e < G; e++) {
      int env = wave * G + e;
      real* bp = nullptr;
      if constexpr (EP >= 2) bp = body_rows(w) + e * kBodyP;
      if constexpr (EP >= 4) env_load<EP>(w.e[e], M, A, env < A.N ? env : A.N - 1, bp, lat_rows(w).late + e * kNU, lat_rows(w).rsw + e, env < A.N, grav_rows(w) + e * kGravP);
      else
      if constexpr (EP >= 3) env_load<EP>(w.e[e], M, A, env < A.N ? env : A.N - 1, bp, lat_rows(w).late + e * kNU, lat_rows(w).rsw + e, env < A.N);
      else
      env_load<EP>(w.e[e], M, A, env < A.N ? env : A.N - 1, bp);
    }
  }
  nm_stamp(0);
  int dropped = 0;
  if (NM_ABLATE(A.ablate) & 1024) return;
  if (!(NM_ABLATE(A.ablate) & 2048))
  for (int s = 0; s < A.nsub; s++) {
    if constexpr (EP >= 3) { if (s > 0) latency_switch(w, s); }
    substep<EP>(w, M, s == A.nsub - 1, &dropped, NM_ABLATE(A.ablate));
  }
  if constexpr (G == 2) {
    if constexpr (EP >= 4) env_finish2<EP>(w, M, src, wave, dropped, published);
    else
    env_finish2(w, M, src, wave, dropped, published);
  } else {
#pragma unroll
    for (int e = 0; e < G; e++) {
      int env = wave * G + e;
      if constexpr (EP >= 4) env_finish<EP>(w.e[e], M, A, env, e == 0 ? dropped : 0, env < A.N, grav_rows(w) + e * kGravP);
      else
      env_finish(w.e[e], M, A, env, e == 0 ? dropped : 0, env < A.N);
    }
  }
  nm_stamp(10);
}

}
```

nightmare_rl_amd/csrc/nm_hip.hip:

```cpp
#include <hip/hip_runtime.h>

#include <cmath>
#include <cstdio>
#include <cstdlib>
#include <cstring>
#include <string>
#include <vector>

#include "../../include/nightmare_hip.h"
#include "nm_host_model.h"
#include "nm_env_loop.h"
#include "nm_env_rows.h"
#include "nm_push.h"
#include "nm_reset_noise.h"
#include "nm_rollout.h"

static thread_local std::string g_err;
static int fail(const std::string& m) { g_err = m; return 1; }
#define HIPCHK(x)                                                                                        \
  do {                                                                                                   \
    hipError_t e_ = (x);                                                                                 \
    if (e_ != hipSuccess) return fail(std::string(#x) + ": " + hipGetErrorString(e_));                  \
  } while (0)

#ifndef NM_WAVES_PER_SIMD
#define NM_WAVES_PER_SIMD 2
#endif
#ifndef NM_ENVS_PER_WAVE
#define NM_ENVS_PER_WAVE 2
#endif
template <class real, class Src> __device__ __noinline__ void step_tail(Src src, real ep_len_s) {
  const nm::Args<real>& A = nm::launch_args(nm::scalar_src(src));
  const int lane = NM_TID;
#define TAIL_LD(p) __hip_atomic_load(p, __ATOMIC_RELAXED, __HIP_MEMORY_SCOPE_AGENT)
  const int cnt = TAIL_LD(A.stat_cnt);
  const int c1 = TAIL_LD(A.stat_cnt + 1), c2 = TAIL_LD(A.stat_cnt + 2);
  const real ssum = TAIL_LD(A.stat_sum + (lane < nm::kNREW ? lane : 0));
  const int n = TAIL_LD(A.nto);
  const int np = TAIL_LD(A.nprev);
  const bool to_full = A.time_outs && TAIL_LD(A.to_owner) != (unsigned long long)(uintptr_t)A.time_outs;
  const long long k0 = lane == 0 ? A.counters[0] : 0, k1 = lane == 0 ? A.counters[1] : 0;
  if (cnt > 0) {
    if (lane < nm::kNREW && A.ep_stats) A.ep_stats[lane] = (float)(ssum / (real)cnt / ep_len_s);
    if (A.time_outs) {
      const int e_new = lane < n ? TAIL_LD(A.to_list + lane) : -1;
      const int e_old = (!to_full && lane < np) ? A.to_prev[lane] : -1;
      if (to_full) {
        for (int i = lane; i < A.N; i += 64) A.time_outs[i] = 0.f;
      } else {
        if (e_old >= 0) A.time_outs[e_old] = 0.f;
        for (int j = lane + 64; j < np; j += 64) A.time_outs[A.to_prev[j]] = 0.f;
      }
      asm volatile("s_waitcnt vmcnt(0)" ::: "memory");
      if (e_new >= 0) { A.time_outs[e_new] = 1.f; A.to_prev[lane] = e_new; }
      for (int j = lane + 64; j < n; j += 64) {
        const int e = TAIL_LD(A.to_list + j);
        A.time_outs[e] = 1.f;
        A.to_prev[j] = e;
      }
      if (lane == 0) { *A.nprev = n; *A.to_owner = (unsigned long long)(uintptr_t)A.time_outs; }
    }
  }
#undef TAIL_LD
  if (lane < nm::kNREW) A.stat_sum[lane] = real(0);
  if (lane == 0) {
    A.counters[0] = k0 + c1;
    A.counters[1] = k1 + c2;
    A.stat_cnt[0] = 0; A.stat_cnt[1] = 0; A.stat_cnt[2] = 0; A.stat_cnt[3] = 0;
    *A.nto = 0;
    A.wave_done[nm::kTicketTop] = 0;
  }
}

#ifdef NM_WG_WAVES
constexpr int kWG = NM_WG_WAVES;
#else
constexpr int kWG = 1;
#endif
struct NoArgsCopy {};
template <class real> __device__ __forceinline__ nm::KernArgs<real, 8> step_src(NoArgsCopy&) { return {(nm::kernarg_ptr)__builtin_amdgcn_kernarg_segment_ptr()}; }
template <class real> __device__ __forceinline__ const nm::Args<real>& step_src(nm::Args<real>& a) { return a; }
template <class real, int G, int EP>
__global__ void __launch_bounds__(64 * (sizeof(real) == 8 ? 1 : kWG), NM_WAVES_PER_SIMD) k_env_step(const nm::Model<real>* __restrict__ Mp, nm::Args<real> A) {
  constexpr int kWG = sizeof(real) == 8 ? 1 : ::kWG;
  static_assert(sizeof(Mp) == 8 && alignof(nm::Args<real>) == 8, "k_env_step: Args starts at byte 8 of the kernarg segment");
  __shared__ typename nm::ShWSel<real, G, EP>::type shs[kWG];
  __shared__ nm::ModelBlock<real> Mb;
  const nm::Model<real>& Ms = Mb.m;
  constexpr bool kKern = sizeof(real) == 4;
  __shared__ std::conditional_t<kKern, NoArgsCopy, nm::Args<real>> As;
  decltype(auto) KA = step_src<real>(As);
  nm::ShW<real, G>& sh = nm::ShWSel<real, G, EP>::images(shs[kWG == 1 ? 0 : (int)(threadIdx.x >> 6)]);
  if constexpr (kKern) nm::launch_args_touch(KA);
  else { As = A; __syncthreads(); }
  int wave;
  unsigned long long t_start = 0ull;
  {
    const nm::Args<real>& A0 = nm::launch_args(KA);
    const int N = A0.N, nxcd = A0.nxcd;
    const bool dbg_on = A0.dbg != nullptr;
#ifdef NM_MEASURE
    if (A0.ablate & 512) return;
#endif
    wave = nmr::wave_index(nxcd);
    if (kWG > 1) wave = wave * kWG + (int)(threadIdx.x >> 6);
    if (dbg_on) t_start = __builtin_amdgcn_s_memtime();
    if (wave * G >= N) return;
  }
  auto copy_model = [&]() {
    typedef uint32_t u4 __attribute__((ext_vector_type(4)));
    constexpr int kRounds = (int)(sizeof(nm::ModelBlock<real>) / (64 * 16));
    const NM_GLOBAL(u4)* src = (const NM_GLOBAL(u4)*)Mp;
    u4* dst = reinterpret_cast<u4*>(&Mb);
    u4 tmp[kRounds];
#pragma unroll
    for (int k = 0; k < kRounds; k++) tmp[k] = src[NM_TID + 64 * k];
    if (kWG == 1 || threadIdx.x < 64) {
#pragma unroll
      for (int k = 0; k < kRounds; k++) dst[NM_TID + 64 * k] = tmp[k];
    }
    if (kWG == 1) nm::wave_sync(); else __syncthreads();
  };
  const int grp = wave / nm::kTicketGroup;
  int ticket = 0, top = 0;
  int stage = 0;
  bool closes_group = false;
  auto draw = [&](int phase) {
#ifdef NM_NO_TICKETS
    stage = 2; (void)phase; return;
#endif
    const nm::Args<real>& Ad = nm::launch_args(KA);
    int* wave_done = Ad.wave_done;
    if (phase == 0) {
      if (NM_TID == 0) ticket = atomicAdd(wave_done + (grp + 1) * nm::kTicketStride, 1);
      stage = 1;
    } else {
      const int nw = (Ad.N + G - 1) / G, gsize = min(nm::kTicketGroup, nw - grp * nm::kTicketGroup);
      closes_group = __builtin_amdgcn_readfirstlane(ticket) == gsize - 1;
      if (closes_group && NM_TID == 0) {
        wave_done[(grp + 1) * nm::kTicketStride] = 0;
        top = atomicAdd(wave_done + nm::kTicketTop, 1);
      }
      stage = 2;
    }
  };
  nm::wave_step<real, G, EP>(sh, Ms, KA, wave, copy_model, draw);
  const nm::Args<real>& A1 = nm::launch_args(KA);
  if (A1.dbg && NM_TID == 0) {
    const unsigned long long t_end = __builtin_amdgcn_s_memtime();
    real* d = A1.dbg + (size_t)(wave * G) * nm::kDbgN + 250;
    d[0] = (real)(unsigned)(t_start & 0xFFFFFF); d[1] = (real)(unsigned)((t_start >> 24) & 0xFFFFFF);
    d[2] = (real)(unsigned)(t_end & 0xFFFFFF); d[3] = (real)(unsigned)((t_end >> 24) & 0xFFFFFF);
    d[4] = (real)(__builtin_amdgcn_s_getreg(4 | (0 << 6) | (15 << 11)) & 0xFFFF);
    d[5] = (real)(__builtin_amdgcn_s_getreg(20 | (0 << 6) | (3 << 11)) & 0xF);
  }
  if (A1.physics_only) return;
  if (stage < 1) draw(0);
  if (stage < 2) draw(1);
  if (!closes_group) return;
  const int ngrp = ((A1.N + G - 1) / G + nm::kTicketGroup - 1) / nm::kTicketGroup;
  if (__builtin_amdgcn_readfirstlane(top) != ngrp - 1) return;
#ifndef NM_SKIP_TAIL2
  if constexpr (kKern) step_tail<real>(KA, Ms.ep_len_s);
  else step_tail<real>(&As, Ms.ep_len_s);
#endif
}


template <class real>
__global__ void k_reset(nm::Model<real> M, nm::Args<real> A, const int32_t* ids, int n) {
  int j = blockIdx.x * blockDim.x + threadIdx.x;
  if (j >= n) return;
  int env = ids ? ids[j] : j;
  for (int k = 0; k < nm::kNQ; k++) A.qpos[env * nm::kNQ + k] = M.qpos0[k];
  for (int k = 0; k < nm::kNV; k++) A.qvel[env * nm::kNV + k] = real(0);
  real ux, uy;
  uint32_t ctr = A.rngctr[env];
  if (A.cmd_u) { ux = A.cmd_u[env * 4 + 2]; uy = A.cmd_u[env * 4 + 3]; }
  else {
    ux = (real)nm::rand_u24_bits(A.seed, (uint64_t)(A.env_offset + env), ctr) * real(1.0 / 16777216.0);
    uy = (real)nm::rand_u24_bits(A.seed, (uint64_t)(A.env_offset + env), ctr + 1) * real(1.0 / 16777216.0);
    ctr += 2;
  }
  real c0 = ux * real(2) * M.max_lin_x - M.max_lin_x, c2 = uy * real(2) * M.max_ang - M.max_ang;
  real keep = sqrt(c0 * c0) > real(0.02) ? real(1) : real(0);
  A.cmd[env * 3] = c0 * keep; A.cmd[env * 3 + 1] = real(0); A.cmd[env * 3 + 2] = c2;
  A.rngctr[env] = ctr;
  A.eplen[env] = 0;
  for (int k = 0; k < nm::kNLEG; k++) A.feetair[env * nm::kNLEG + k] = real(0);
  for (int k = 0; k < nm::kNREW; k++) {
    atomicAdd(A.stat_sum + k, A.epsum[env * nm::kNREW + k]);
    A.epsum[env * nm::kNREW + k] = real(0);
  }
  atomicAdd(A.stat_cnt, 1);
}

template <class real>
__global__ void k_finalize(int N, real* stat_sum, int* stat_cnt, float* ep_stats, const float* timeout_now, float* time_outs,
                           real ep_len_s, long long* counters) {
// ... 93 lines not shown
  virtual void set_ablate(int m) = 0;
  virtual int set_noise(const double* vec) = 0;
  virtual int set_noise_u(const double* u) = 0;
  virtual int set_record(int idx) = 0;
  virtual int get_record(double* qpos, double* qvel, int32_t* nbad) = 0;
  virtual int play(const nm_play_args* r, int act, hipStream_t s) = 0;
  virtual int tape(const nm_tape_args* r, hipStream_t s) = 0;
  virtual int get_log(int first, int count, double* rows) = 0;
  virtual int get_log_dones(int first, int count, unsigned char* dones) = 0;
  virtual int set_env_params(const void* mu, const void* p_gain, const void* kv, hipStream_t s) = 0;
  virtual int get_env_params(void* mu, void* p_gain, void* kv, hipStream_t s) = 0;
  virtual int draw_env_params(const double* lo, const double* hi, hipStream_t s) = 0;
  virtual int set_body_params(const void* rows, hipStream_t s) = 0;
  virtual int get_body_params(void* out, hipStream_t s) = 0;
  virtual int draw_payload(const double* lo, const double* hi, void* out, hipStream_t s) = 0;
  virtual int set_action_latency(const int* substeps, hipStream_t s) = 0;
  virtual int get_action_latency(int* out, hipStream_t s) = 0;
  virtual int draw_action_latency(int lo, int hi, hipStream_t s) = 0;
  virtual int set_action_history(const float* h, hipStream_t s) = 0;
  virtual int get_action_history(float* out, hipStream_t s) = 0;
  virtual int set_gravity(const void* rows, hipStream_t s) = 0;
  virtual int get_gravity(void* out, hipStream_t s) = 0;
  virtual int draw_gravity(const double* lo, const double* hi, void* out, hipStream_t s) = 0;
  virtual int set_servo(const void* rows, hipStream_t s) = 0;
  virtual int get_servo(void* out, hipStream_t s) = 0;
  virtual int draw_servo(const double* lo, const double* hi, hipStream_t s) = 0;
  virtual int get_servo_state(double* L) = 0;
  virtual int set_servo_state(const double* L) = 0;
  int push_interval = 0;
  double push_max = 0.0;
  uint64_t push_step = 0;
  int rnoise_on = 0;
  double rnoise_ranges[2 * nm::kResetRanges] = {};
  virtual int set_reset_counts(const uint32_t* counts_host) = 0;
  virtual int get_reset_counts(uint32_t* counts_host) = 0;
};

template <class real> struct Env : nm_env {
  nmhost::Tables<real> T;
  nm::Model<real> M;
  nm::Args<real> A;
  std::vector<void*> allocs;
  real* cmd_u_dev = nullptr;
  bool cmd_u_on = false;
  float* timeout_now = nullptr;
  int32_t* ids_dev = nullptr;
  long long* counters_dev = nullptr;
  nm::Model<real>* M_dev = nullptr;
  real* noise_vec_dev = nullptr;
  real* noise_u_dev = nullptr;
  bool noise_on = false, noise_u_on = false;
  uint64_t noise_step = 0;
  real* rec_dev = nullptr;
  int rec_env = -1;
  real* rec_log = nullptr;
  int rec_log_cap = 0, rec_log_rows = 0;
  unsigned char* rec_done = nullptr;
  bool rec_done_valid = false;
  const real* rec_last = nullptr;
  bool prof_on = false;
  std::vector<std::pair<hipEvent_t, hipEvent_t>> prof_ev;
  size_t prof_used = 0;

  char* slab = nullptr;
  size_t slab_size = 0, slab_used = 0;
  int slab_init(size_t bytes) {
// ... 98 lines not shown
    if (!physics_only && (!eplen || !obs || !rew || !done)) return fail("nm_step: NULL output pointer");
    nm::Args<real> a = A;
    a.actions = actions; a.eplen = eplen; a.obs = obs; a.rew = rew; a.done = done; a.timeout_now = timeout_now;
    a.cmd_u = cmd_u_on ? cmd_u_dev : nullptr;
    a.physics_only = physics_only;
    a.ep_stats = ep_stats; a.time_outs = time_outs; a.counters = counters_dev;
    if (!physics_only) {
      a.noise_vec = noise_on ? noise_vec_dev : nullptr;
      a.noise_u = noise_on && noise_u_on ? noise_u_dev : nullptr;
      a.noise_step = noise_step++;
      a.rec = rec_env >= 0 ? rec_dev : nullptr;
      a.rec_env = rec_env;
      if (rec_env >= 0) rec_last = rec_dev;
      const uint64_t ps = push_step++;
      if (nm::push_due(push_interval, ps)) {
        hipLaunchKernelGGL(nm::k_push<real>, dim3((2 * N + 255) / 256), dim3(256), 0, s, A.qvel, N, A.seed, A.env_offset,
                           nm::push_counter(push_interval, ps), (real)push_max);
        HIPCHK(hipGetLastError());
      }
    }
    hipEvent_t e0 = nullptr, e1 = nullptr;
    if (prof_on) {
      if (prof_used == prof_ev.size()) {
        HIPCHK(hipEventCreate(&e0));
        HIPCHK(hipEventCreate(&e1));
        prof_ev.push_back({e0, e1});
      }
      e0 = prof_ev[prof_used].first; e1 = prof_ev[prof_used].second;
      prof_used++;
      HIPCHK(hipEventRecord(e0, s));
    }
    constexpr int G = sizeof(real) == 8 ? 1 : NM_ENVS_PER_WAVE;
    constexpr int W = sizeof(real) == 8 ? 1 : kWG;
    nmrows::with_level5(rows.level(physics_only), [&](auto L) {
      hipLaunchKernelGGL((k_env_step<real, G, decltype(L)::value>), dim3((N + G * W - 1) / (G * W)), dim3(64 * W), 0, s, (const nm::Model<real>*)M_dev, a);
    });
    HIPCHK(hipGetLastError());
    if (prof_on) HIPCHK(hipEventRecord(e1, s));
    if (!physics_only && rnoise_on && launch_reset_noise(done, nullptr, N, s)) return 1;
    return 0;
  }
  int d2h(const real* dev, double* host, size_t n) {
    if (!host) return 0;
    std::vector<real> tmp(n);
    HIPCHK(hipMemcpy(tmp.data(), dev, n * sizeof(real), hipMemcpyDeviceToHost));
    for (size_t i = 0; i < n; i++) host[i] = (double)tmp[i];
    return 0;
  }
  int h2d(real* dev, const double* host, size_t n) {
    if (!host) return 0;
    std::vector<real> tmp(n);
    for (size_t i = 0; i < n; i++) tmp[i] = (real)host[i];
    HIPCHK(hipMemcpy(dev, tmp.data(), n * sizeof(real), hipMemcpyHostToDevice));
    return 0;
  }
  int get_state(double* qpos, double* qvel, double* qw) override {
    HIPCHK(hipSetDevice(device));
    HIPCHK(hipDeviceSynchronize());
    return d2h(A.qpos, qpos, (size_t)N * 25) || d2h(A.qvel, qvel, (size_t)N * 24) || d2h(A.qwarm, qw, (size_t)N * 24);
  }
  int set_state(const double* qpos, const double* qvel, const double* qw) override {
    HIPCHK(hipSetDevice(device));
    HIPCHK(hipDeviceSynchronize());
    return h2d(A.qpos, qpos, (size_t)N * 25) || h2d(A.qvel, qvel, (size_t)N * 24) || h2d(A.qwarm, qw, (size_t)N * 24);
  }
  int get_buffers(double* dp, double* dv, double* act, double* cmd, double* es) override {
    HIPCHK(hipSetDevice(device));
    HIPCHK(hipDeviceSynchronize());
    return d2h(A.dofpos, dp, (size_t)N * 18) || d2h(A.dofvel, dv, (size_t)N * 18) || d2h(A.act, act, (size_t)N * 18) ||
           d2h(A.cmd, cmd, (size_t)N * 3) || d2h(A.epsum, es, (size_t)N * nm::kNREW);
// ... 771 lines not shown
  return env->get_servo(out_dev, (hipStream_t)stream);
}
int nm_draw_servo(nm_env* env, const double lo[2], const double hi[2], void* stream) {
  static const char* kCol[2] = {"rate", "d_gain"};
  const auto extra = [](int k, double lo_k) -> const char* {
    return k == 0 ? (lo_k > 0.0 ? nullptr : "rate must be above 0") : (lo_k < 0.0 ? "d_gain must not be negative" : nullptr);
  };
  if (draw_bounds_bad("nm_draw_servo", env, lo, hi, kCol, 2, extra, false, nullptr)) return 1;
  if (env->dtype == NM_DTYPE_F32 && !((float)lo[0] > 0.0f)) return fail("nm_draw_servo: rate must be above 0 in float32");
  return env->draw_servo(lo, hi, (hipStream_t)stream);
}
int nm_get_servo_state(nm_env* env, double* limited) {
  NEED_ENV(env);
  return env->get_servo_state(limited);
}
int nm_set_servo_state(nm_env* env, const double* limited) {
  NEED_ENV(env);
  return env->set_servo_state(limited);
}
int nm_step_tape(nm_env* env, const nm_tape_args* args, void* stream) {
  if (!env) return fail("nm_step_tape: env is NULL");
  if (!args) return fail("nm_step_tape: args is NULL");
  return env->tape(args, (hipStream_t)stream);
}
#ifdef NM_STAMPS
int nm_read_stamps(unsigned long long* out16, int reset) {
  (void)hipDeviceSynchronize();
  if (out16 && hipMemcpyFromSymbol(out16, HIP_SYMBOL(nm::g_stamps), 16 * sizeof(unsigned long long)) != hipSuccess) return fail("nm_read_stamps: copy failed");
  unsigned long long z[16] = {0};
  if (reset && hipMemcpyToSymbol(HIP_SYMBOL(nm::g_stamps), z, sizeof z) != hipSuccess) return fail("nm_read_stamps: reset failed");
  return 0;
}
#endif
int nm_profile(nm_env* env, int32_t enable, double* sum_ms, int64_t* count) { NEED(env); return env->profiling(enable, sum_ms, count); }
}
```

nightmare_rl_amd/csrc/simt.h:

```cpp
#pragma once
#include <stdint.h>

#define NM_WAVE 64

#ifndef NM_EMUL
#include <hip/hip_runtime.h>
#define NM_FN __device__ __forceinline__
#define NM_HDFN __host__ __device__ __forceinline__
#define NM_COLD __device__ __noinline__
namespace simt {
template <class T> using V = T;
using VB = bool;

#ifdef NM_WG_WAVES
#define NM_TID ((int)(threadIdx.x & 63))
#else
#define NM_TID ((int)threadIdx.x)
#endif
NM_FN int lane_id() { return NM_TID; }
template <class T> NM_FN T sel(bool c, T a, T b) { return c ? a : b; }
NM_FN float vsqrt(float x) { return sqrtf(x); }
NM_FN double vsqrt(double x) { return sqrt(x); }
NM_FN float vabs(float x) { return fabsf(x); }
NM_FN double vabs(double x) { return fabs(x); }
// ... 2 lines not shown
NM_FN float vmin(float a, float b) { return fminf(a, b); }
NM_FN double vmin(double a, double b) { return fmin(a, b); }
NM_FN int vmin(int a, int b) { return a < b ? a : b; }
NM_FN int vmax(int a, int b) { return a > b ? a : b; }
NM_FN void vsincos(float x0, float* s, float* c) {
  const float x = fminf(fmaxf(x0, -4194304.0f), 4194304.0f);
  const float k = rintf(x * 0.636619772f);
  float r = fmaf(-k, 1.5707963705062866f, x);
  r = fmaf(-k, -4.371139000186241e-8f, r);
  const float r2 = r * r;
  const float ps = fmaf(r * r2, fmaf(r2, fmaf(r2, -1.9515295891e-4f, 8.3321608736e-3f), -1.6666654611e-1f), r);
  const float pc = fmaf(r2 * r2, fmaf(r2, fmaf(r2, 2.443315711809948e-5f, -1.388731625493765e-3f), 4.166664568298827e-2f), fmaf(r2, -0.5f, 1.0f));
  const int n = (int)k;
  const float sa = (n & 1) ? pc : ps, ca = (n & 1) ? ps : pc;
  *s = (n & 2) ? -sa : sa;
  *c = ((n + 1) & 2) ? -ca : ca;
}
NM_FN void vsincos(double x, double* s, double* c) { sincos(x, s, c); }
NM_FN float vexp(float x) { return expf(x); }
NM_FN double vexp(double x) { return exp(x); }
NM_FN float vacos(float x) { return acosf(x); }
NM_FN double vacos(double x) { return acos(x); }
NM_FN float vpow(float x, float p) { return powf(x, p); }
NM_FN double vpow(double x, double p) { return pow(x, p); }
NM_FN bool visbad(float x) { return !(fabsf(x) <= 1e10f); }
NM_FN bool visbad(double x) { return !(fabs(x) <= 1e10); }
template <class T> NM_FN T to_real(int i) { return (T)i; }
template <class T, class S> NM_FN T vcvt(S x) { return (T)x; }
NM_FN float vrcp(float x) { return __builtin_amdgcn_rcpf(x); }
NM_FN double vrcp(double x) { return 1.0 / x; }

NM_FN float vfma(float a, float b, float c) { return __builtin_fmaf(a, b, c); }
NM_FN double vfma(double a, double b, double c) { return __builtin_fma(a, b, c); }
NM_FN float sel_mask(uint64_t m, float a, float b) {
  float r;
  asm("v_cndmask_b32_e64 %0, %1, %2, %3" : "=v"(r) : "v"(b), "v"(a), "s"(m));
  return r;
}
NM_FN double sel_mask(uint64_t m, double a, double b) {
  int rl, rh;
  asm("v_cndmask_b32_e64 %0, %2, %3, %6\n\tv_cndmask_b32_e64 %1, %4, %5, %6" : "=&v"(rl), "=v"(rh)
      : "v"(__double2loint(b)), "v"(__double2loint(a)), "v"(__double2hiint(b)), "v"(__double2hiint(a)), "s"(m));
  return __hiloint2double(rh, rl);
}
NM_FN uint64_t mask_shl(uint64_t m, int k) { m <<= k; asm("" : "+s"(m)); return m; }
template <int I> NM_FN float fma_half_lane(float a, float x, float g, bool h1);
template <int I> NM_FN double fma_half_lane(double a, double x, double g, bool h1);
NM_FN int rdlane(int x, int l) { return __builtin_amdgcn_readlane(x, l); }
NM_FN float rdlane(float x, int l) { return __int_as_float(__builtin_amdgcn_readlane(__float_as_int(x), l)); }
NM_FN double rdlane(double x, int l) {
  int lo = __builtin_amdgcn_readlane(__double2loint(x), l), hi = __builtin_amdgcn_readlane(__double2hiint(x), l);
  return __hiloint2double(hi, lo);
}
template <int I> NM_FN float fma_half_lane(float a, float x, float g, bool h1) {
  const float s0 = rdlane(x, I), s1 = rdlane(x, 32 + I);
  return vfma(a, h1 ? s1 : s0, g);
}
template <int I> NM_FN double fma_half_lane(double a, double x, double g, bool h1) {
  const double s0 = rdlane(x, I), s1 = rdlane(x, 32 + I);
  return vfma(a, h1 ? s1 : s0, g);
}
template <class T> NM_FN T wrlane(T x, T v, int l) {
  int ln = NM_TID;
  asm volatile("" : "+v"(ln));
  return ln == l ? v : x;
}
// ... 148 lines not shown
#define NM_SEL(T)                                                                                              \
  NM_FN V<T> sel(const VB& c, const V<T>& a, const V<T>& b) { V<T> r; for (int i = 0; i < NM_WAVE; i++) r.v[i] = c.v[i] ? a.v[i] : b.v[i]; return r; } \
  NM_FN T sel(bool c, T a, T b) { return c ? a : b; }
NM_SEL(float) NM_SEL(double) NM_SEL(int)
#undef NM_SEL
#define NM_MAP1(name, expr)                                                                                   \
  NM_FN V<float> name(const V<float>& a) { V<float> r; for (int i = 0; i < NM_WAVE; i++) { float x = a.v[i]; r.v[i] = expr; } return r; } \
  NM_FN V<double> name(const V<double>& a) { V<double> r; for (int i = 0; i < NM_WAVE; i++) { double x = a.v[i]; r.v[i] = expr; } return r; } \
  NM_FN float name(float x) { return expr; }                                                                  \
  NM_FN double name(double x) { return expr; }
NM_MAP1(vsqrt, std::sqrt(x)) NM_MAP1(vabs, std::fabs(x)) NM_MAP1(vexp, std::exp(x)) NM_MAP1(vacos, std::acos(x))
#undef NM_MAP1
#define NM_MAP2(name, expr, T)                                                                               \
  NM_FN V<T> name(const V<T>& a, const V<T>& b) { V<T> r; for (int i = 0; i < NM_WAVE; i++) { T x = a.v[i], y = b.v[i]; r.v[i] = expr; } return r; } \
  NM_FN T name(T x, T y) { return expr; }
NM_MAP2(vmax, (x > y ? x : y), float) NM_MAP2(vmax, (x > y ? x : y), double) NM_MAP2(vmax, (x > y ? x : y), int)
NM_MAP2(vmin, (x < y ? x : y), float) NM_MAP2(vmin, (x < y ? x : y), double) NM_MAP2(vmin, (x < y ? x : y), int)
NM_MAP2(vpow, std::pow(x, y), float) NM_MAP2(vpow, std::pow(x, y), double)
#undef NM_MAP2
template <class T> NM_FN void vsincos(const V<T>& x, V<T>* s, V<T>* c) { for (int i = 0; i < NM_WAVE; i++) { s->v[i] = std::sin(x.v[i]); c->v[i] = std::cos(x.v[i]); } }
NM_FN void vsincos(float x, float* s, float* c) { *s = std::sin(x); *c = std::cos(x); }
NM_FN void vsincos(double x, double* s, double* c) { *s = std::sin(x); *c = std::cos(x); }
template <class T> NM_FN VB visbad(const V<T>& a) { VB r; for (int i = 0; i < NM_WAVE; i++) r.v[i] = !(std::fabs(a.v[i]) <= (T)1e10); return r; }
NM_FN bool visbad(float x) { return !(std::fabs(x) <= 1e10f); }
NM_FN bool visbad(double x) { return !(std::fabs(x) <= 1e10); }
template <class T> NM_FN V<T> to_real(const V<int>& a) { V<T> r; for (int i = 0; i < NM_WAVE; i++) r.v[i] = (T)a.v[i]; return r; }
template <class T> NM_FN T to_real(int a) { return (T)a; }
template <class T> NM_FN V<T> vrcp(const V<T>& a) { V<T> r; for (int i = 0; i < NM_WAVE; i++) r.v[i] = (T)1 / a.v[i]; return r; }
NM_FN float vrcp(float x) { return 1.0f / x; }
NM_FN double vrcp(double x) { return 1.0 / x; }
template <class T, class S> NM_FN V<T> vcvt(const V<S>& a) { V<T> r; for (int i = 0; i < NM_WAVE; i++) r.v[i] = (T)a.v[i]; return r; }

template <class T> NM_FN V<T> vfma(const V<T>& a, const V<T>& b, const V<T>& c) { return a * b + c; }
NM_FN float vfma(float a, float b, float c) { return a * b + c; }
NM_FN double vfma(double a, double b, double c) { return a * b + c; }
template <class T> NM_FN V<T> sel_mask(uint64_t m, const V<T>& a, const V<T>& b) {
  V<T> r;
  for (int i = 0; i < NM_WAVE; i++) r.v[i] = ((m >> i) & 1ull) ? a.v[i] : b.v[i];
  return r;
}
NM_FN uint64_t mask_shl(uint64_t m, int k) { return m << k; }
template <int I, class T> NM_FN V<T> fma_half_lane(const V<T>& a, const V<T>& x, const V<T>& g, const VB&) {
  V<T> r;
  for (int i = 0; i < NM_WAVE; i++) r.v[i] = a.v[i] * x.v[(i & 32) + I] + g.v[i];
  return r;
}
template <class T> NM_FN T rdlane(const V<T>& x, int l) { return x.v[l]; }
template <class T> NM_FN T rdlane(T x, int) { return x; }
template <class T> NM_FN V<T> wrlane(V<T> x, T v, int l) { x.v[l] = v; return x; }
NM_FN V<int> opaque_lane() { return lane_id(); }
template <class T> NM_FN T uniform(const V<T>& x) { return x.v[0]; }
template <class T> NM_FN T uniform(T x) { return x; }
template <class T> NM_FN V<T> shfl_xor(const V<T>& x, int m) { V<T> r; for (int i = 0; i < NM_WAVE; i++) r.v[i] = x.v[i ^ m]; return r; }
template <int P, class T> NM_FN V<T> quad(const V<T>& x) { V<T> r; for (int i = 0; i < NM_WAVE; i++) r.v[i] = x.v[(i & ~3) | ((P >> (2 * (i & 3))) & 3)]; return r; }
template <class T> NM_FN V<T> shfl_xor1(const V<T>& x) { return shfl_xor(x, 1); }
template <class T> NM_FN V<T> shfl_xor2(const V<T>& x) { return shfl_xor(x, 2); }
template <class T> NM_FN V<T> half_mirror(const V<T>& x) { V<T> r; for (int i = 0; i < NM_WAVE; i++) r.v[i] = x.v[(i & ~7) | (7 - (i & 7))]; return r; }
template <class T> NM_FN V<T> row_mirror(const V<T>& x) { V<T> r; for (int i = 0; i < NM_WAVE; i++) r.v[i] = x.v[(i & ~15) | (15 - (i & 15))]; return r; }
template <class T> NM_FN V<T> gsum8(V<T> x) {
  x = x + shfl_xor(x, 1); x = x + shfl_xor(x, 2); x = x + half_mirror(x);
  return x;
}
template <class T> NM_FN T wsum8(V<T> x) {
  x = x + shfl_xor(x, 1); x = x + shfl_xor(x, 2); x = x + half_mirror(x);
  return x.v[0];
}
// ... 51 lines not shown
```

nightmare_rl_amd/envs/nightmare_v3_env.py:

```python
import ctypes as C
import numpy as np
import torch

from .. import _lib
from .helpers import class_to_dict
from .nightmare_v3_config import NightmareV3Config
from .state_log import ROW as _LOG_ROW, StateLog


def push_config(cfg, dt):
    dr = getattr(cfg, "domain_rand", None)
    if dr is None or not getattr(dr, "push_robots", False):
        return 0, 0.0
    steps = float(dr.push_interval_s) / float(dt) + 1e-9
    if not steps >= 1:
        raise ValueError("cfg.domain_rand.push_interval_s must be at least one env step (dt)")
    vel = float(dr.max_push_vel_xy)
    if not (vel >= 0 and np.isfinite(vel)):
        raise ValueError("cfg.domain_rand.max_push_vel_xy must be finite and >= 0")
    if steps >= 2 ** 31:
        raise ValueError("cfg.domain_rand.push_interval_s is more than 2^31 env steps")
    return int(steps), vel


# ... 750 lines not shown
        arrs = [None if a is None else np.ascontiguousarray(a, np.float64) for a in (dof_pos, dof_vel, actions, commands, episode_sums)]
        self._ck(self._L.nm_set_buffers(self._h, *[None if a is None else a.ctypes.data for a in arrs]))

    def get_feet_state(self):
        N = self.num_envs
        air, last, filt = np.empty((N, 6)), np.empty((N, 6), np.uint8), np.empty((N, 6), np.uint8)
        self._ck(self._L.nm_get_feet_state(self._h, air.ctypes.data, last.ctypes.data, filt.ctypes.data))
        return air, last, filt

    def set_feet_state(self, air=None, last=None, filt=None):
        f = lambda a, t: None if a is None else np.ascontiguousarray(a, t)
        arrs = [f(air, np.float64), f(last, np.uint8), f(filt, np.uint8)]
        self._ck(self._L.nm_set_feet_state(self._h, *[None if a is None else a.ctypes.data for a in arrs]))

    def set_command_uniforms(self, u):
        a = None if u is None else np.ascontiguousarray(u, np.float64).reshape(self.num_envs, 4)
        self._ck(self._L.nm_set_command_uniforms(self._h, None if a is None else a.ctypes.data))

    def counters(self):
        out = np.zeros(3, np.int64)
        self._ck(self._L.nm_get_counters(self._h, out.ctypes.data))
        return dict(contacts_dropped=int(out[0]), bad_state_resets=int(out[1]), hull_search_fallbacks=int(out[2]))

    def set_debug_buffer(self, t):
        self._dbg = t
        self._ck(self._L.nm_set_debug_buffer(self._h, None if t is None else t.data_ptr()))

    def accumulate_rewards_into(self, t):
        if t is not None and (t.dtype != torch.float32 or t.numel() != self.num_envs or not t.is_contiguous() or t.device != self.obs_buf.device):
            raise ValueError("accumulate_rewards_into: contiguous float32 [num_envs] tensor on the env's device")
        self._ret_acc = t
        self._ck(self._L.nm_set_return_accumulator(self._h, None if t is None else t.data_ptr()))

    def profile(self, enable):
        ms, cnt = C.c_double(0), C.c_int64(0)
        self._ck(self._L.nm_profile(self._h, int(bool(enable)), C.byref(ms), C.byref(cnt)))
        return ms.value, cnt.value

    @property
    def commands(self):
        return self.get_buffers()["commands"]

    def close(self):
        if getattr(self, "_h", None) is not None and self._h:
            torch.cuda.synchronize(self.device)
            self._L.nm_destroy(self._h)
            self._h = None

    def __del__(self):
        try:
            self.close()
        except Exception:
            pass
```

Before: 86.42 million env-steps/s.

## Add compile-time specialized lean step kernel for default configuration

Introduces a CfgLean policy that fixes model and argument options (link rotation ids, square softness, contact modes, batch threshold, no debug/record/noise/cmd_u/physics_only) as constexpr, and templates the step pipeline on it. A separate lean kernel instantiation is launched when the runtime config matches, so branches and optional loads become dead code and register pressure may drop. It adds a second kernel variant, a runtime selection switch, and rounding-pinned subtractions to keep results bitwise equal to the generic path.

```diff
diff --git a/include/nightmare_hip.h b/include/nightmare_hip.h
--- a/include/nightmare_hip.h
+++ b/include/nightmare_hip.h
@@ -99,6 +99,8 @@
 int nm_get_state_log_dones(nm_env* env, int32_t first_step, int32_t count, unsigned char* dones_host);
 
 int nm_profile(nm_env* env, int32_t enable, double* sum_ms, int64_t* count);
+int nm_set_step_variant(nm_env* env, int32_t mode);
+int nm_get_step_variant(nm_env* env);
 
 typedef enum {
   NM_ACT_ELU = 0,
diff --git a/nightmare_rl_amd/_lib.py b/nightmare_rl_amd/_lib.py
--- a/nightmare_rl_amd/_lib.py
+++ b/nightmare_rl_amd/_lib.py
@@ -28,7 +28,8 @@
            "nm_set_action_latency", "nm_get_action_latency", "nm_draw_action_latency", "nm_set_action_history", "nm_get_action_history",
            "nm_set_reset_noise", "nm_get_reset_noise", "nm_reset_noise_offsets",
            "nm_set_gravity", "nm_get_gravity", "nm_draw_gravity",
-           "nm_set_servo", "nm_get_servo", "nm_draw_servo", "nm_get_servo_state", "nm_set_servo_state"]
+           "nm_set_servo", "nm_get_servo", "nm_draw_servo", "nm_get_servo_state", "nm_set_servo_state",
+           "nm_set_step_variant", "nm_get_step_variant"]
 
 
 class NmConfig(C.Structure):
@@ -189,6 +190,9 @@
         L.nm_draw_servo.argtypes = [vp, C.POINTER(C.c_double * 2), C.POINTER(C.c_double * 2), vp]
         L.nm_get_servo_state.argtypes = [vp, vp]
         L.nm_set_servo_state.argtypes = [vp, vp]
+    if hasattr(L, "nm_set_step_variant"):
+        L.nm_set_step_variant.argtypes = [vp, C.c_int32]
+        L.nm_get_step_variant.argtypes = [vp]
     if not full:
         return L
     L.nm_gae.argtypes = [vp, vp, vp, vp, C.c_int32, C.c_int32, C.c_float, C.c_float, vp, vp]
diff --git a/nightmare_rl_amd/csrc/nm_core.h b/nightmare_rl_amd/csrc/nm_core.h
--- a/nightmare_rl_amd/csrc/nm_core.h
+++ b/nightmare_rl_amd/csrc/nm_core.h
@@ -152,6 +152,43 @@
 }
 #endif
 
+struct CfgAsk { static constexpr bool kLean = false; };
+struct CfgLean {
+  static constexpr bool kLean = true;
+  static constexpr int kTibiaMode = 1, kBodyMode = 1, kBatchMin = 3;
+  static constexpr bool link_rot_id(int k) { return k != 0; }
+};
+template <class Cfg, class real> NM_FN bool cfg_link_rot_id(const Model<real>& M, int k) {
+  if constexpr (Cfg::kLean) return Cfg::link_rot_id(k); else return uniform(M.link_rot_id[k]);
+}
+template <class Cfg, class real> NM_FN bool cfg_si_square(const Model<real>& M) {
+  if constexpr (Cfg::kLean) return true; else return M.si_power == real(2);
+}
+template <class Cfg, class real> NM_FN int cfg_tibia_mode(const Model<real>& M) {
+  if constexpr (Cfg::kLean) return Cfg::kTibiaMode; else return M.tibia_mode;
+}
+template <class Cfg, class real> NM_FN int cfg_body_mode(const Model<real>& M) {
+  if constexpr (Cfg::kLean) return Cfg::kBodyMode; else return M.body_mode;
+}
+template <class Cfg, class real> NM_FN int cfg_rew_extra(const Model<real>& M) {
+  if constexpr (Cfg::kLean) return 0; else return M.rew_extra;
+}
+template <class Cfg, class real> NM_FN int cfg_batch_min(const Model<real>& M) {
+  if constexpr (Cfg::kLean) return Cfg::kBatchMin; else return M.collide_batch_min;
+}
+template <class Cfg, class T> NM_FN T* cfg_opt(T* p) {
+  if constexpr (Cfg::kLean) return nullptr; else return p;
+}
+template <class Cfg> NM_FN int cfg_flag(int f) {
+  if constexpr (Cfg::kLean) return 0; else return f;
+}
+template <class real> inline bool lean_config(const Model<real>& M, const Args<real>& A) {
+  for (int k = 0; k < 3; k++)
+    if ((M.link_rot_id[k] != 0) != CfgLean::link_rot_id(k)) return false;
+  return M.si_power == real(2) && M.tibia_mode == CfgLean::kTibiaMode && M.body_mode == CfgLean::kBodyMode && M.rew_extra == 0 &&
+         M.collide_batch_min == CfgLean::kBatchMin && !A.dbg && !A.rec && !A.noise_vec && !A.cmd_u && !A.physics_only && !A.ablate;
+}
+
 template <class real> struct Sh {
   real qpos[kNQ];
   real envp[kEnvPS];
@@ -430,7 +467,7 @@
   return gsum8(sel(isleg, x, V<real>(real(0))));
 }
 
-template <int EP, class real, int G> NM_FN void stage_smooth(ShW<real, G>& w, const Model<real>& M, bool last) {
+template <int EP, class real, int G, class Cfg = CfgAsk> NM_FN void stage_smooth(ShW<real, G>& w, const Model<real>& M, bool last, Cfg = Cfg()) {
   typedef V<real> vr;
   real* lds = reinterpret_cast<real*>(&w.e[0]);
   static_assert((G & (G - 1)) == 0 && 2 * G <= 8, "lane groups: G envs x 2 factorisations");
@@ -528,7 +565,7 @@
         vr ax[3] = {ldsv(M.legc, cb + 12), ldsv(M.legc, cb + 13), ldsv(M.legc, cb + 14)};
         vr R0[9];
         {
-          if (uniform(M.link_rot_id[k])) {
+          if (cfg_link_rot_id<Cfg>(M, k)) {
 #pragma unroll
             for (int j = 0; j < 9; j++) R0[j] = Rp[j];
           } else {
@@ -1214,7 +1251,7 @@
     hull_ring(M, vadr + r.cur[g], r.nb[g], r.vv[g]);
   }
 }
-template <class real> NM_FN void stage_collide(Sh<real>& sh, const Model<real>& M, int* dropped, Rings<real>& rg, bool pairs = true) {
+template <class real, class Cfg = CfgAsk> NM_FN void stage_collide(Sh<real>& sh, const Model<real>& M, int* dropped, Rings<real>& rg, bool pairs = true, Cfg = Cfg()) {
   typedef V<real> vr;
   const V<int> lane = lane_id();
   const real bz = sh.qpos[2];
@@ -1291,7 +1328,7 @@
   for (int g = 0; g < kNCOL; g++) hitbits |= (uniform(near[g] && pz[g] - sv[g] < real(0)) ? 1u : 0u) << g;
   const int nhit = popc64(hitbits);
   bool batch = false;
-  if (nhit >= M.collide_batch_min) {
+  if (nhit >= cfg_batch_min<Cfg>(M)) {
     const uint64_t hitm = (uint64_t)hitbits << kBatchLane0;
     vr X[3] = {vv[kNCOL - 1][0], vv[kNCOL - 1][1], vv[kNCOL - 1][2]}, svl = val[kNCOL - 1];
     V<int> slackl = nb[kNCOL - 1];
@@ -1428,7 +1465,7 @@
 template <class X> NM_FN X noslip_pair_cost(const X& d, const X& hK1, const X& dg) { return d * vfma(hK1, d, dg); }
 template <class real, class X> NM_FN auto noslip_pair_bad(const X& change) { return change > X(real(1e-10)); }
 
-template <class real, bool PAIR, int EP> NM_FN void stage_constraint_body(Sh<real>& sh, real* jrow, const Model<real>& M, bool last, bool nosweep, BodyRef<EP, real> br) {
+template <class real, bool PAIR, int EP, class Cfg = CfgAsk> NM_FN void stage_constraint_body(Sh<real>& sh, real* jrow, const Model<real>& M, bool last, bool nosweep, BodyRef<EP, real> br) {
   typedef V<real> vr;
   const V<int> lane = lane_id();
   const int ncon = uniform(sh.ncon), nefc = 4 * ncon;
@@ -1548,10 +1585,10 @@
   {
     vr x = vabs(dist) * vrcp(M.si_width);
     vr ylo, yhi;
-    if (M.si_power == real(2)) {
-      vr omx = vmax(vr(real(1)) - x, vr(real(0)));
+    if (cfg_si_square<Cfg>(M)) {
+      vr omx = vmax(vsub_rn(vr(real(1)), x), vr(real(0)));
       ylo = (x * x) * vrcp(M.si_mid);
-      yhi = vr(real(1)) - (omx * omx) * vrcp(real(1) - M.si_mid);
+      yhi = vsub_rn(vr(real(1)), (omx * omx) * vrcp(real(1) - M.si_mid));
     } else {
       ylo = vpow(x, vr(M.si_power)) / vpow(vr(M.si_mid), vr(M.si_power - real(1)));
       yhi = vr(real(1)) - vpow(vmax(vr(real(1)) - x, vr(real(0))), vr(M.si_power)) / vpow(vr(real(1) - M.si_mid), vr(M.si_power - real(1)));
@@ -1803,15 +1840,15 @@
   wave_sync();
 }
 
-template <class real, int EP> NM_COLD void stage_constraint_pairs(Sh<real>& sh, real* jrow, const Model<real>& M, bool last, bool nosweep, BodyRef<EP, real> br) {
-  stage_constraint_body<real, true, EP>(sh, jrow, M, last, nosweep, br);
+template <class real, int EP, class Cfg = CfgAsk> NM_COLD void stage_constraint_pairs(Sh<real>& sh, real* jrow, const Model<real>& M, bool last, bool nosweep, BodyRef<EP, real> br) {
+  stage_constraint_body<real, true, EP, Cfg>(sh, jrow, M, last, nosweep, br);
 }
 
 constexpr int kMaxCon2 = 8, kMaxRow2 = 4 * kMaxCon2;
 #ifdef NM_EMUL
 inline long& nm_emul_together() { static long n = 0; return n; }
 #endif
-template <int EP, class real> NM_FN void stage_constraint2(ShW<real, 2>& w, const Model<real>& M, bool last, bool nosweep) {
+template <int EP, class real, class Cfg = CfgAsk> NM_FN void stage_constraint2(ShW<real, 2>& w, const Model<real>& M, bool last, bool nosweep, Cfg = Cfg()) {
   typedef V<real> vr;
   constexpr int kSR = (int)(sizeof(Sh<real>) / sizeof(real)), kSI = (int)(sizeof(Sh<real>) / sizeof(int));
   const V<int> lane = lane_id();
@@ -1902,10 +1939,10 @@
   {
     vr x = vabs(dist) * vrcp(M.si_width);
     vr ylo, yhi;
-    if (M.si_power == real(2)) {
-      vr omx = vmax(vr(real(1)) - x, vr(real(0)));
+    if (cfg_si_square<Cfg>(M)) {
+      vr omx = vmax(vsub_rn(vr(real(1)), x), vr(real(0)));
       ylo = (x * x) * vrcp(M.si_mid);
-      yhi = vr(real(1)) - (omx * omx) * vrcp(real(1) - M.si_mid);
+      yhi = vsub_rn(vr(real(1)), (omx * omx) * vrcp(real(1) - M.si_mid));
     } else {
       ylo = vpow(x, vr(M.si_power)) / vpow(vr(M.si_mid), vr(M.si_power - real(1)));
       yhi = vr(real(1)) - vpow(vmax(vr(real(1)) - x, vr(real(0))), vr(M.si_power)) / vpow(vr(real(1) - M.si_mid), vr(M.si_power - real(1)));
@@ -2501,10 +2538,10 @@
   stsv(sh.cnrm(), c * 3 + 2, V<real>(real(1)), on);
   wave_sync();
 }
-template <class real, int EP> NM_FN void stage_constraint(Sh<real>& sh, real* jrow, const Model<real>& M, bool last, bool nosweep, BodyRef<EP, real> br) {
+template <class real, int EP, class Cfg = CfgAsk> NM_FN void stage_constraint(Sh<real>& sh, real* jrow, const Model<real>& M, bool last, bool nosweep, BodyRef<EP, real> br) {
   if (uniform(sh.ncon) > kMaxCon) { floor_frames(sh); stage_constraint_big<real, EP>(sh, M, last, nosweep, br); }
-  else if (uniform(sh.anypair) != 0) { floor_frames(sh); stage_constraint_pairs<real, EP>(sh, jrow, M, last, nosweep, br); }
-  else stage_constraint_body<real, false, EP>(sh, jrow, M, last, nosweep, br);
+  else if (uniform(sh.anypair) != 0) { floor_frames(sh); stage_constraint_pairs<real, EP, Cfg>(sh, jrow, M, last, nosweep, br); }
+  else stage_constraint_body<real, false, EP, Cfg>(sh, jrow, M, last, nosweep, br);
 }
 
 template <class real, int G, int EP = 0> NM_FN void stage_integrate(ShW<real, G>& w, const Model<real>& M) {
@@ -2663,7 +2700,7 @@
 inline void nm_set_priority(int) {}
 #endif
 
-template <int EP, class real, int G> NM_FN void substep(ShW<real, G>& w, const Model<real>& M, bool last, int* dropped, int ablate) {
+template <int EP, class real, int G, class Cfg = CfgAsk> NM_FN void substep(ShW<real, G>& w, const Model<real>& M, bool last, int* dropped, int ablate, Cfg cfg = Cfg()) {
   const V<int> lane = opaque_lane();
   if constexpr (G == 2) {
     constexpr int kSR = (int)(sizeof(Sh<real>) / sizeof(real));
@@ -2691,11 +2728,11 @@
   }
   wave_sync();
   nm_stamp(1);
-  if (!(ablate & 8)) stage_smooth<EP>(w, M, last);
+  if (!(ablate & 8)) stage_smooth<EP>(w, M, last, cfg);
   nm_stamp(2);
   for (int e = 0; e < G; e++) {
     Sh<real>& sh = w.e[e];
-    if (!(ablate & 1)) { Rings<real> rg; collide_rings(sh, M, rg); stage_collide(sh, M, dropped, rg, G != 2 && !(ablate & 16)); }
+    if (!(ablate & 1)) { Rings<real> rg; collide_rings(sh, M, rg); stage_collide(sh, M, dropped, rg, G != 2 && !(ablate & 16), cfg); }
     else { sh.ncon = 0; sh.anypair = 0; wave_sync(); }
   }
   if constexpr (G == 2) {
@@ -2714,7 +2751,7 @@
       nm_emul_together() += 1;
 #endif
       w.e[0].ntog += 1;
-      stage_constraint2<EP>(w, M, last, (ablate & 2) != 0);
+      stage_constraint2<EP>(w, M, last, (ablate & 2) != 0, cfg);
       nm_stamp(8);
     }
   }
@@ -2722,7 +2759,7 @@
     for (int e = 0; e < G; e++) {
       BodyRef<EP, real> br;
       if constexpr (EP >= 2) br = BodyRef<EP, real>(body_rows(w) + e * kBodyP);
-      stage_constraint<real, EP>(w.e[e], w.jrow, M, last, (ablate & 2) != 0, br);
+      stage_constraint<real, EP, Cfg>(w.e[e], w.jrow, M, last, (ablate & 2) != 0, br);
       nm_stamp(8);
     }
   if constexpr (EP >= 4) stage_integrate<real, G, EP>(w, M);
@@ -3120,7 +3157,7 @@
 }
 
 struct NoMid { NM_FN void operator()() const {} NM_FN void operator()(int) const {} };
-template <int EP, class real, class Src, class Mid> NM_FN void env_load2(ShW<real, 2>& w, const Model<real>& M, const Src& src, int wave, Mid&& mid) {
+template <int EP, class real, class Src, class Mid, class Cfg = CfgAsk> NM_FN void env_load2(ShW<real, 2>& w, const Model<real>& M, const Src& src, int wave, Mid&& mid, Cfg = Cfg()) {
   typedef V<real> vr;
   const Args<real>& A = launch_args(src);
   constexpr bool kS = ArgSrc<Src>::kScalarBase;
@@ -3149,7 +3186,7 @@
   V<int> dl = V<int>(0);
   V<float> h0 = V<float>(0.0f), h1 = V<float>(0.0f), h2 = V<float>(0.0f);
   if constexpr (EP >= 3)
-    if (!A.physics_only) {
+    if (!cfg_flag<Cfg>(A.physics_only)) {
       dl = gldx<kS>(lat_delay(A), env);
       h0 = gldx<kS>(lat_hist(A), l18c + env * (kLatH * kNU));
       h1 = gldx<kS>(lat_hist(A), l18c + (env * (kLatH * kNU) + kNU));
@@ -3157,7 +3194,7 @@
     }
   vr servo_in = vr(real(0)), lim_in = vr(real(0));
   if constexpr (EP >= 5)
-    if (!A.physics_only) {
+    if (!cfg_flag<Cfg>(A.physics_only)) {
       servo_in = gldx<kS>(servo_rows_of(A), sel(hl < kServoP, hl, V<int>(0)) + env * kServoP);
       lim_in = gldx<kS>(servo_state_of(A), l18c + env * kNU);
     }
@@ -3165,7 +3202,7 @@
   int64_t ep = 0;
   uint32_t ctr_in = 0;
 #endif
-  if (!A.physics_only) {
+  if (!cfg_flag<Cfg>(A.physics_only)) {
     cmd_in = gldx<kS>(A.cmd, sel(hl < 3, hl, V<int>(0)) + env * 3);
     eps_in = gldx<kS>(A.epsum, sel(hl < kNREW, hl, V<int>(0)) + env * kNREW);
 #ifndef NM_EMUL
@@ -3205,7 +3242,7 @@
 #else
   act = (real)af;
 #endif
-  if (!A.physics_only) {
+  if (!cfg_flag<Cfg>(A.physics_only)) {
     stsv(rb, ho + (hl + NM_OFS(ecmd)), cmd_in, hl < 3);
     stsv(rb, ho + (hl + NM_OFS(eepsum)), eps_in, hl < kNREW);
 #ifdef NM_EMUL
@@ -3256,7 +3293,7 @@
   wave_sync();
 }
 
-template <int EP = 0, class real, class Src, class Pub> NM_FN void env_finish2(ShW<real, 2>& w, const Model<real>& M, const Src& src, int wave, int dropped, Pub&& published) {
+template <int EP = 0, class real, class Src, class Pub, class Cfg = CfgAsk> NM_FN void env_finish2(ShW<real, 2>& w, const Model<real>& M, const Src& src, int wave, int dropped, Pub&& published, Cfg = Cfg()) {
   typedef V<real> vr;
   const Args<real>& A = launch_args(src);
   constexpr bool kS = ArgSrc<Src>::kScalarBase;
@@ -3290,14 +3327,14 @@
     gstx<kS>(A.qpos, hl + env * kNQ, q, live & (hl < kNQ));
     gstx<kS>(A.qvel, hl + env * kNV, v, live & (hl < kNV));
     gstx<kS>(A.qwarm, hl + env * kNV, wq, live & (hl < kNV));
-    if (A.rec) {
+    if (cfg_opt<Cfg>(A.rec)) {
       const VB r = live & (env == V<int>(A.rec_env));
       gstx<kS>(A.rec, hl, q, r & (hl < kNQ));
       gstx<kS>(A.rec, hl + kNQ, v, r & (hl < kNV));
       gstx<kS>(A.rec, V<int>(kNQ + kNV), to_real<real>(nwarn), r & (hl == 0));
     }
   }
-  if (A.dbg) {
+  if (cfg_opt<Cfg>(A.dbg)) {
     if (lives[0]) env_debug(w.e[0], A, wave * 2, dropped);
     if (lives[1]) env_debug(w.e[1], A, wave * 2 + 1, 0);
   }
@@ -3310,7 +3347,7 @@
     if (hl == 0 && live && nwarn) nm_consume(atomicAdd(A.stat_cnt + 2, nwarn));
 #endif
   }
-  if (A.physics_only) return;
+  if (cfg_flag<Cfg>(A.physics_only)) return;
   if (NM_ABLATE(A.ablate) & 128) return;
   NM_ESTAMP(11);
 
@@ -3350,7 +3387,7 @@
   auto resample = [&](int hh, int which) {
     const int e = wave * 2 + hh;
     real ux, uy;
-    if (A.cmd_u) { ux = gld1(A.cmd_u, (size_t)(e * 4 + 2 * which)); uy = gld1(A.cmd_u, (size_t)(e * 4 + 2 * which + 1)); }
+    if (cfg_opt<Cfg>(A.cmd_u)) { ux = gld1(A.cmd_u, (size_t)(e * 4 + 2 * which)); uy = gld1(A.cmd_u, (size_t)(e * 4 + 2 * which + 1)); }
     else {
       ux = (real)rand_u24_bits(A.seed, (uint64_t)(A.env_offset + e), ctr[hh]) * real(1.0 / 16777216.0);
       uy = (real)rand_u24_bits(A.seed, (uint64_t)(A.env_offset + e), ctr[hh] + 1) * real(1.0 / 16777216.0);
@@ -3382,12 +3419,12 @@
 #pragma unroll
     for (int l = 1; l < 6; l++) fm = vmax(fm, feet[l]);
     reset = reset | (fm > vr(M.term_force));
-    if ((M.tibia_mode == 2) | (M.body_mode == 2)) {
+    if ((cfg_tibia_mode<Cfg>(M) == 2) | (cfg_body_mode<Cfg>(M) == 2)) {
       vr tm = tib[0];
 #pragma unroll
       for (int l = 1; l < 6; l++) tm = vmax(tm, tib[l]);
-      if (M.tibia_mode == 2) reset = reset | (tm > vr(M.tibia_max));
-      if (M.body_mode == 2) reset = reset | (body > vr(M.body_max));
+      if (cfg_tibia_mode<Cfg>(M) == 2) reset = reset | (tm > vr(M.tibia_max));
+      if (cfg_body_mode<Cfg>(M) == 2) reset = reset | (body > vr(M.body_max));
     }
     vr nrm = vsqrt(pg[0] * pg[0] + pg[1] * pg[1] + pg[2] * pg[2]);
     if (sizeof(real) == 8) reset = reset | (vacos(-pg[2] / nrm) > vr(real(1.0471975511965976)));
@@ -3427,9 +3464,9 @@
     vr da = prev_act - act;
     rt[R_ACTION_RATE] = hsum32(sel(l18, da * da, vr(real(0)))) * M.rew_scale[R_ACTION_RATE];
     vr sumt = ((tib[0] + tib[1]) + (tib[2] + tib[3])) + (tib[4] + tib[5]);
-    if ((M.tibia_mode != 1) | (M.body_mode != 1)) {
-      sumt = M.tibia_mode == 1 ? sumt : vr(real(0));
-      body = M.body_mode == 1 ? body : vr(real(0));
+    if ((cfg_tibia_mode<Cfg>(M) != 1) | (cfg_body_mode<Cfg>(M) != 1)) {
+      sumt = cfg_tibia_mode<Cfg>(M) == 1 ? sumt : vr(real(0));
+      body = cfg_body_mode<Cfg>(M) == 1 ? body : vr(real(0));
     }
     rt[R_BODY_CONTACT] = (sumt + body) * M.rew_scale[R_BODY_CONTACT];
     vr dp = dofpos - defp;
@@ -3442,7 +3479,7 @@
     vr el = (cmd[0] - blv[0]) * (cmd[0] - blv[0]) + (cmd[1] - blv[1]) * (cmd[1] - blv[1]);
     rt[R_TRACK_LIN] = vexp(-el / M.sigma) * M.rew_scale[R_TRACK_LIN];
     rt[R_TERMINATION] = sel(reset & !time_out, vr(M.rew_scale[R_TERMINATION]), vr(real(0)));
-    if (M.rew_extra) {
+    if (cfg_rew_extra<Cfg>(M)) {
       rt[R_ANG_VEL_XY] = (bav[0] * bav[0] + bav[1] * bav[1]) * M.rew_scale[R_ANG_VEL_XY];
       vr dh = SHR(bh, V<int>(0)) - M.base_h_target;
       rt[R_BASE_HEIGHT] = dh * dh * M.rew_scale[R_BASE_HEIGHT];
@@ -3493,7 +3530,7 @@
     auto put = [&](const vr& x0, const V<int>& idx, const VB& m0) {
       const VB m = m0 & live;
       vr x = x0;
-      if (A.noise_vec) {
+      if (cfg_opt<Cfg>(A.noise_vec)) {
         auto nz = [&](int k, int e) {
           real u = A.noise_u ? gld1(A.noise_u, (size_t)e * kNOBS + k)
                              : (real)rand_u24_bits(A.seed + kNoiseKey, (uint64_t)(A.env_offset + e), (uint32_t)(A.noise_step * kNOBS + k)) * real(1.0 / 16777216.0);
@@ -3566,12 +3603,13 @@
   wave_sync();
 }
 
-template <class real, int G, int EP = 0, class Mid = NoMid, class Pub = NoMid, class Src = Args<real>>
-NM_FN void wave_step(ShW<real, G>& w, const Model<real>& M, const Src& src, int wave, Mid&& mid = Mid(), Pub&& published = Pub()) {
+template <class real, int G, int EP = 0, class Mid = NoMid, class Pub = NoMid, class Src = Args<real>, class Cfg = CfgAsk>
+NM_FN void wave_step(ShW<real, G>& w, const Model<real>& M, const Src& src, int wave, Mid&& mid = Mid(), Pub&& published = Pub(), Cfg cfg = Cfg()) {
+  static_assert(!Cfg::kLean || G == 2, "CfgLean: the one-env stages (env_load, env_finish) ask at run time");
   const Args<real>& A = launch_args(src);
   nm_stamp(-1);
   if constexpr (G == 2) {
-    env_load2<EP>(w, M, src, wave, mid);
+    env_load2<EP>(w, M, src, wave, mid, cfg);
   } else {
     mid();
 #pragma unroll
@@ -3592,12 +3630,12 @@
   if (!(NM_ABLATE(A.ablate) & 2048))
   for (int s = 0; s < A.nsub; s++) {
     if constexpr (EP >= 3) { if (s > 0) latency_switch(w, s); }
-    substep<EP>(w, M, s == A.nsub - 1, &dropped, NM_ABLATE(A.ablate));
+    substep<EP>(w, M, s == A.nsub - 1, &dropped, NM_ABLATE(A.ablate), cfg);
   }
   if constexpr (G == 2) {
-    if constexpr (EP >= 4) env_finish2<EP>(w, M, src, wave, dropped, published);
+    if constexpr (EP >= 4) env_finish2<EP>(w, M, src, wave, dropped, published, cfg);
     else
-    env_finish2(w, M, src, wave, dropped, published);
+    env_finish2(w, M, src, wave, dropped, published, cfg);
   } else {
 #pragma unroll
     for (int e = 0; e < G; e++) {
diff --git a/nightmare_rl_amd/csrc/nm_hip.hip b/nightmare_rl_amd/csrc/nm_hip.hip
--- a/nightmare_rl_amd/csrc/nm_hip.hip
+++ b/nightmare_rl_amd/csrc/nm_hip.hip
@@ -23,148 +23,7 @@
     if (e_ != hipSuccess) return fail(std::string(#x) + ": " + hipGetErrorString(e_));                  \
   } while (0)
 
-#ifndef NM_WAVES_PER_SIMD
-#define NM_WAVES_PER_SIMD 2
-#endif
-#ifndef NM_ENVS_PER_WAVE
-#define NM_ENVS_PER_WAVE 2
-#endif
-template <class real, class Src> __device__ __noinline__ void step_tail(Src src, real ep_len_s) {
-  const nm::Args<real>& A = nm::launch_args(nm::scalar_src(src));
-  const int lane = NM_TID;
-#define TAIL_LD(p) __hip_atomic_load(p, __ATOMIC_RELAXED, __HIP_MEMORY_SCOPE_AGENT)
-  const int cnt = TAIL_LD(A.stat_cnt);
-  const int c1 = TAIL_LD(A.stat_cnt + 1), c2 = TAIL_LD(A.stat_cnt + 2);
-  const real ssum = TAIL_LD(A.stat_sum + (lane < nm::kNREW ? lane : 0));
-  const int n = TAIL_LD(A.nto);
-  const int np = TAIL_LD(A.nprev);
-  const bool to_full = A.time_outs && TAIL_LD(A.to_owner) != (unsigned long long)(uintptr_t)A.time_outs;
-  const long long k0 = lane == 0 ? A.counters[0] : 0, k1 = lane == 0 ? A.counters[1] : 0;
-  if (cnt > 0) {
-    if (lane < nm::kNREW && A.ep_stats) A.ep_stats[lane] = (float)(ssum / (real)cnt / ep_len_s);
-    if (A.time_outs) {
-      const int e_new = lane < n ? TAIL_LD(A.to_list + lane) : -1;
-      const int e_old = (!to_full && lane < np) ? A.to_prev[lane] : -1;
-      if (to_full) {
-        for (int i = lane; i < A.N; i += 64) A.time_outs[i] = 0.f;
-      } else {
-        if (e_old >= 0) A.time_outs[e_old] = 0.f;
-        for (int j = lane + 64; j < np; j += 64) A.time_outs[A.to_prev[j]] = 0.f;
-      }
-      asm volatile("s_waitcnt vmcnt(0)" ::: "memory");
-      if (e_new >= 0) { A.time_outs[e_new] = 1.f; A.to_prev[lane] = e_new; }
-      for (int j = lane + 64; j < n; j += 64) {
-        const int e = TAIL_LD(A.to_list + j);
-        A.time_outs[e] = 1.f;
-        A.to_prev[j] = e;
-      }
-      if (lane == 0) { *A.nprev = n; *A.to_owner = (unsigned long long)(uintptr_t)A.time_outs; }
-    }
-  }
-#undef TAIL_LD
-  if (lane < nm::kNREW) A.stat_sum[lane] = real(0);
-  if (lane == 0) {
-    A.counters[0] = k0 + c1;
-    A.counters[1] = k1 + c2;
-    A.stat_cnt[0] = 0; A.stat_cnt[1] = 0; A.stat_cnt[2] = 0; A.stat_cnt[3] = 0;
-    *A.nto = 0;
-    A.wave_done[nm::kTicketTop] = 0;
-  }
-}
-
-#ifdef NM_WG_WAVES
-constexpr int kWG = NM_WG_WAVES;
-#else
-constexpr int kWG = 1;
-#endif
-struct NoArgsCopy {};
-template <class real> __device__ __forceinline__ nm::KernArgs<real, 8> step_src(NoArgsCopy&) { return {(nm::kernarg_ptr)__builtin_amdgcn_kernarg_segment_ptr()}; }
-template <class real> __device__ __forceinline__ const nm::Args<real>& step_src(nm::Args<real>& a) { return a; }
-template <class real, int G, int EP>
-__global__ void __launch_bounds__(64 * (sizeof(real) == 8 ? 1 : kWG), NM_WAVES_PER_SIMD) k_env_step(const nm::Model<real>* __restrict__ Mp, nm::Args<real> A) {
-  constexpr int kWG = sizeof(real) == 8 ? 1 : ::kWG;
-  static_assert(sizeof(Mp) == 8 && alignof(nm::Args<real>) == 8, "k_env_step: Args starts at byte 8 of the kernarg segment");
-  __shared__ typename nm::ShWSel<real, G, EP>::type shs[kWG];
-  __shared__ nm::ModelBlock<real> Mb;
-  const nm::Model<real>& Ms = Mb.m;
-  constexpr bool kKern = sizeof(real) == 4;
-  __shared__ std::conditional_t<kKern, NoArgsCopy, nm::Args<real>> As;
-  decltype(auto) KA = step_src<real>(As);
-  nm::ShW<real, G>& sh = nm::ShWSel<real, G, EP>::images(shs[kWG == 1 ? 0 : (int)(threadIdx.x >> 6)]);
-  if constexpr (kKern) nm::launch_args_touch(KA);
-  else { As = A; __syncthreads(); }
-  int wave;
-  unsigned long long t_start = 0ull;
-  {
-    const nm::Args<real>& A0 = nm::launch_args(KA);
-    const int N = A0.N, nxcd = A0.nxcd;
-    const bool dbg_on = A0.dbg != nullptr;
-#ifdef NM_MEASURE
-    if (A0.ablate & 512) return;
-#endif
-    wave = nmr::wave_index(nxcd);
-    if (kWG > 1) wave = wave * kWG + (int)(threadIdx.x >> 6);
-    if (dbg_on) t_start = __builtin_amdgcn_s_memtime();
-    if (wave * G >= N) return;
-  }
-  auto copy_model = [&]() {
-    typedef uint32_t u4 __attribute__((ext_vector_type(4)));
-    constexpr int kRounds = (int)(sizeof(nm::ModelBlock<real>) / (64 * 16));
-    const NM_GLOBAL(u4)* src = (const NM_GLOBAL(u4)*)Mp;
-    u4* dst = reinterpret_cast<u4*>(&Mb);
-    u4 tmp[kRounds];
-#pragma unroll
-    for (int k = 0; k < kRounds; k++) tmp[k] = src[NM_TID + 64 * k];
-    if (kWG == 1 || threadIdx.x < 64) {
-#pragma unroll
-      for (int k = 0; k < kRounds; k++) dst[NM_TID + 64 * k] = tmp[k];
-    }
-    if (kWG == 1) nm::wave_sync(); else __syncthreads();
-  };
-  const int grp = wave / nm::kTicketGroup;
-  int ticket = 0, top = 0;
-  int stage = 0;
-  bool closes_group = false;
-  auto draw = [&](int phase) {
-#ifdef NM_NO_TICKETS
-    stage = 2; (void)phase; return;
-#endif
-    const nm::Args<real>& Ad = nm::launch_args(KA);
-    int* wave_done = Ad.wave_done;
-    if (phase == 0) {
-      if (NM_TID == 0) ticket = atomicAdd(wave_done + (grp + 1) * nm::kTicketStride, 1);
-      stage = 1;
-    } else {
-      const int nw = (Ad.N + G - 1) / G, gsize = min(nm::kTicketGroup, nw - grp * nm::kTicketGroup);
-      closes_group = __builtin_amdgcn_readfirstlane(ticket) == gsize - 1;
-      if (closes_group && NM_TID == 0) {
-        wave_done[(grp + 1) * nm::kTicketStride] = 0;
-        top = atomicAdd(wave_done + nm::kTicketTop, 1);
-      }
-      stage = 2;
-    }
-  };
-  nm::wave_step<real, G, EP>(sh, Ms, KA, wave, copy_model, draw);
-  const nm::Args<real>& A1 = nm::launch_args(KA);
-  if (A1.dbg && NM_TID == 0) {
-    const unsigned long long t_end = __builtin_amdgcn_s_memtime();
-    real* d = A1.dbg + (size_t)(wave * G) * nm::kDbgN + 250;
-    d[0] = (real)(unsigned)(t_start & 0xFFFFFF); d[1] = (real)(unsigned)((t_start >> 24) & 0xFFFFFF);
-    d[2] = (real)(unsigned)(t_end & 0xFFFFFF); d[3] = (real)(unsigned)((t_end >> 24) & 0xFFFFFF);
-    d[4] = (real)(__builtin_amdgcn_s_getreg(4 | (0 << 6) | (15 << 11)) & 0xFFFF);
-    d[5] = (real)(__builtin_amdgcn_s_getreg(20 | (0 << 6) | (3 << 11)) & 0xF);
-  }
-  if (A1.physics_only) return;
-  if (stage < 1) draw(0);
-  if (stage < 2) draw(1);
-  if (!closes_group) return;
-  const int ngrp = ((A1.N + G - 1) / G + nm::kTicketGroup - 1) / nm::kTicketGroup;
-  if (__builtin_amdgcn_readfirstlane(top) != ngrp - 1) return;
-#ifndef NM_SKIP_TAIL2
-  if constexpr (kKern) step_tail<real>(KA, Ms.ep_len_s);
-  else step_tail<real>(&As, Ms.ep_len_s);
-#endif
-}
+#include "nm_step_kernel.h"
 
 
 template <class real>
@@ -324,6 +183,7 @@
   uint64_t push_step = 0;
   int rnoise_on = 0;
   double rnoise_ranges[2 * nm::kResetRanges] = {};
+  int step_variant_mode = 0, step_variant_last = 0;
   virtual int set_reset_counts(const uint32_t* counts_host) = 0;
   virtual int get_reset_counts(uint32_t* counts_host) = 0;
 };
@@ -488,10 +348,22 @@
     }
     constexpr int G = sizeof(real) == 8 ? 1 : NM_ENVS_PER_WAVE;
     constexpr int W = sizeof(real) == 8 ? 1 : kWG;
-    nmrows::with_level5(rows.level(physics_only), [&](auto L) {
-      hipLaunchKernelGGL((k_env_step<real, G, decltype(L)::value>), dim3((N + G * W - 1) / (G * W)), dim3(64 * W), 0, s, (const nm::Model<real>*)M_dev, a);
-    });
-    HIPCHK(hipGetLastError());
+    bool lean = false;
+#ifndef NM_MEASURE
+    if constexpr (sizeof(real) == 4 && G == 2)
+      lean = step_variant_mode == 0 && rows.level(physics_only) == 0 && nm::lean_config(M, a);
+#endif
+    step_variant_last = lean ? 1 : 0;
+    if (lean) {
+#ifndef NM_MEASURE
+      if constexpr (sizeof(real) == 4 && G == 2) HIPCHK(nm_launch_step_lean(N, s, (const nm::Model<float>*)M_dev, a));
+#endif
+    } else {
+      nmrows::with_level5(rows.level(physics_only), [&](auto L) {
+        hipLaunchKernelGGL((k_env_step<real, G, decltype(L)::value>), dim3((N + G * W - 1) / (G * W)), dim3(64 * W), 0, s, (const nm::Model<real>*)M_dev, a);
+      });
+      HIPCHK(hipGetLastError());
+    }
     if (prof_on) HIPCHK(hipEventRecord(e1, s));
     if (!physics_only && rnoise_on && launch_reset_noise(done, nullptr, N, s)) return 1;
     return 0;
@@ -1329,5 +1201,12 @@
   return 0;
 }
 #endif
+int nm_set_step_variant(nm_env* env, int32_t mode) {
+  NEED(env);
+  if (mode != 0 && mode != 1) return fail("nm_set_step_variant: mode must be 0 (choose per launch) or 1 (always the generic kernel)");
+  env->step_variant_mode = mode;
+  return 0;
+}
+int nm_get_step_variant(nm_env* env) { return env ? env->step_variant_last : 0; }
 int nm_profile(nm_env* env, int32_t enable, double* sum_ms, int64_t* count) { NEED(env); return env->profiling(enable, sum_ms, count); }
 }
diff --git a/nightmare_rl_amd/csrc/nm_step_kernel.h b/nightmare_rl_amd/csrc/nm_step_kernel.h
--- /dev/null
+++ b/nightmare_rl_amd/csrc/nm_step_kernel.h
@@ -0,0 +1,150 @@
+#pragma once
+#include <hip/hip_runtime.h>
+
+#include "nm_core.h"
+#include "nm_env_loop.h"
+
+#ifndef NM_WAVES_PER_SIMD
+#define NM_WAVES_PER_SIMD 2
+#endif
+#ifndef NM_ENVS_PER_WAVE
+#define NM_ENVS_PER_WAVE 2
+#endif
+template <class real, class Src> __device__ __noinline__ void step_tail(Src src, real ep_len_s) {
+  const nm::Args<real>& A = nm::launch_args(nm::scalar_src(src));
+  const int lane = NM_TID;
+#define TAIL_LD(p) __hip_atomic_load(p, __ATOMIC_RELAXED, __HIP_MEMORY_SCOPE_AGENT)
+  const int cnt = TAIL_LD(A.stat_cnt);
+  const int c1 = TAIL_LD(A.stat_cnt + 1), c2 = TAIL_LD(A.stat_cnt + 2);
+  const real ssum = TAIL_LD(A.stat_sum + (lane < nm::kNREW ? lane : 0));
+  const int n = TAIL_LD(A.nto);
+  const int np = TAIL_LD(A.nprev);
+  const bool to_full = A.time_outs && TAIL_LD(A.to_owner) != (unsigned long long)(uintptr_t)A.time_outs;
+  const long long k0 = lane == 0 ? A.counters[0] : 0, k1 = lane == 0 ? A.counters[1] : 0;
+  if (cnt > 0) {
+    if (lane < nm::kNREW && A.ep_stats) A.ep_stats[lane] = (float)(ssum / (real)cnt / ep_len_s);
+    if (A.time_outs) {
+      const int e_new = lane < n ? TAIL_LD(A.to_list + lane) : -1;
+      const int e_old = (!to_full && lane < np) ? A.to_prev[lane] : -1;
+      if (to_full) {
+        for (int i = lane; i < A.N; i += 64) A.time_outs[i] = 0.f;
+      } else {
+        if (e_old >= 0) A.time_outs[e_old] = 0.f;
+        for (int j = lane + 64; j < np; j += 64) A.time_outs[A.to_prev[j]] = 0.f;
+      }
+      asm volatile("s_waitcnt vmcnt(0)" ::: "memory");
+      if (e_new >= 0) { A.time_outs[e_new] = 1.f; A.to_prev[lane] = e_new; }
+      for (int j = lane + 64; j < n; j += 64) {
+        const int e = TAIL_LD(A.to_list + j);
+        A.time_outs[e] = 1.f;
+        A.to_prev[j] = e;
+      }
+      if (lane == 0) { *A.nprev = n; *A.to_owner = (unsigned long long)(uintptr_t)A.time_outs; }
+    }
+  }
+#undef TAIL_LD
+  if (lane < nm::kNREW) A.stat_sum[lane] = real(0);
+  if (lane == 0) {
+    A.counters[0] = k0 + c1;
+    A.counters[1] = k1 + c2;
+    A.stat_cnt[0] = 0; A.stat_cnt[1] = 0; A.stat_cnt[2] = 0; A.stat_cnt[3] = 0;
+    *A.nto = 0;
+    A.wave_done[nm::kTicketTop] = 0;
+  }
+}
+
+#ifdef NM_WG_WAVES
+constexpr int kWG = NM_WG_WAVES;
+#else
+constexpr int kWG = 1;
+#endif
+struct NoArgsCopy {};
+template <class real> __device__ __forceinline__ nm::KernArgs<real, 8> step_src(NoArgsCopy&) { return {(nm::kernarg_ptr)__builtin_amdgcn_kernarg_segment_ptr()}; }
+template <class real> __device__ __forceinline__ const nm::Args<real>& step_src(nm::Args<real>& a) { return a; }
+template <class real, int G, int EP, class Cfg = nm::CfgAsk>
+__global__ void __launch_bounds__(64 * (sizeof(real) == 8 ? 1 : kWG), NM_WAVES_PER_SIMD) k_env_step(const nm::Model<real>* __restrict__ Mp, nm::Args<real> A) {
+  constexpr int kWG = sizeof(real) == 8 ? 1 : ::kWG;
+  static_assert(sizeof(Mp) == 8 && alignof(nm::Args<real>) == 8, "k_env_step: Args starts at byte 8 of the kernarg segment");
+  __shared__ typename nm::ShWSel<real, G, EP>::type shs[kWG];
+  __shared__ nm::ModelBlock<real> Mb;
+  const nm::Model<real>& Ms = Mb.m;
+  constexpr bool kKern = sizeof(real) == 4;
+  __shared__ std::conditional_t<kKern, NoArgsCopy, nm::Args<real>> As;
+  decltype(auto) KA = step_src<real>(As);
+  nm::ShW<real, G>& sh = nm::ShWSel<real, G, EP>::images(shs[kWG == 1 ? 0 : (int)(threadIdx.x >> 6)]);
+  if constexpr (kKern) nm::launch_args_touch(KA);
+  else { As = A; __syncthreads(); }
+  int wave;
+  unsigned long long t_start = 0ull;
+  {
+    const nm::Args<real>& A0 = nm::launch_args(KA);
+    const int N = A0.N, nxcd = A0.nxcd;
+    const bool dbg_on = nm::cfg_opt<Cfg>(A0.dbg) != nullptr;
+#ifdef NM_MEASURE
+    if (A0.ablate & 512) return;
+#endif
+    wave = nmr::wave_index(nxcd);
+    if (kWG > 1) wave = wave * kWG + (int)(threadIdx.x >> 6);
+    if (dbg_on) t_start = __builtin_amdgcn_s_memtime();
+    if (wave * G >= N) return;
+  }
+  auto copy_model = [&]() {
+    typedef uint32_t u4 __attribute__((ext_vector_type(4)));
+    constexpr int kRounds = (int)(sizeof(nm::ModelBlock<real>) / (64 * 16));
+    const NM_GLOBAL(u4)* src = (const NM_GLOBAL(u4)*)Mp;
+    u4* dst = reinterpret_cast<u4*>(&Mb);
+    u4 tmp[kRounds];
+#pragma unroll
+    for (int k = 0; k < kRounds; k++) tmp[k] = src[NM_TID + 64 * k];
+    if (kWG == 1 || threadIdx.x < 64) {
+#pragma unroll
+      for (int k = 0; k < kRounds; k++) dst[NM_TID + 64 * k] = tmp[k];
+    }
+    if (kWG == 1) nm::wave_sync(); else __syncthreads();
+  };
+  const int grp = wave / nm::kTicketGroup;
+  int ticket = 0, top = 0;
+  int stage = 0;
+  bool closes_group = false;
+  auto draw = [&](int phase) {
+#ifdef NM_NO_TICKETS
+    stage = 2; (void)phase; return;
+#endif
+    const nm::Args<real>& Ad = nm::launch_args(KA);
+    int* wave_done = Ad.wave_done;
+    if (phase == 0) {
+      if (NM_TID == 0) ticket = atomicAdd(wave_done + (grp + 1) * nm::kTicketStride, 1);
+      stage = 1;
+    } else {
+      const int nw = (Ad.N + G - 1) / G, gsize = min(nm::kTicketGroup, nw - grp * nm::kTicketGroup);
+      closes_group = __builtin_amdgcn_readfirstlane(ticket) == gsize - 1;
+      if (closes_group && NM_TID == 0) {
+        wave_done[(grp + 1) * nm::kTicketStride] = 0;
+        top = atomicAdd(wave_done + nm::kTicketTop, 1);
+      }
+      stage = 2;
+    }
+  };
+  nm::wave_step<real, G, EP>(sh, Ms, KA, wave, copy_model, draw, Cfg());
+  const nm::Args<real>& A1 = nm::launch_args(KA);
+  if (nm::cfg_opt<Cfg>(A1.dbg) && NM_TID == 0) {
+    const unsigned long long t_end = __builtin_amdgcn_s_memtime();
+    real* d = A1.dbg + (size_t)(wave * G) * nm::kDbgN + 250;
+    d[0] = (real)(unsigned)(t_start & 0xFFFFFF); d[1] = (real)(unsigned)((t_start >> 24) & 0xFFFFFF);
+    d[2] = (real)(unsigned)(t_end & 0xFFFFFF); d[3] = (real)(unsigned)((t_end >> 24) & 0xFFFFFF);
+    d[4] = (real)(__builtin_amdgcn_s_getreg(4 | (0 << 6) | (15 << 11)) & 0xFFFF);
+    d[5] = (real)(__builtin_amdgcn_s_getreg(20 | (0 << 6) | (3 << 11)) & 0xF);
+  }
+  if (nm::cfg_flag<Cfg>(A1.physics_only)) return;
+  if (stage < 1) draw(0);
+  if (stage < 2) draw(1);
+  if (!closes_group) return;
+  const int ngrp = ((A1.N + G - 1) / G + nm::kTicketGroup - 1) / nm::kTicketGroup;
+  if (__builtin_amdgcn_readfirstlane(top) != ngrp - 1) return;
+#ifndef NM_SKIP_TAIL2
+  if constexpr (kKern) step_tail<real>(KA, Ms.ep_len_s);
+  else step_tail<real>(&As, Ms.ep_len_s);
+#endif
+}
+
+hipError_t nm_launch_step_lean(int N, hipStream_t s, const nm::Model<float>* M_dev, const nm::Args<float>& a);
diff --git a/nightmare_rl_amd/csrc/nm_step_lean.hip b/nightmare_rl_amd/csrc/nm_step_lean.hip
--- /dev/null
+++ b/nightmare_rl_amd/csrc/nm_step_lean.hip
@@ -0,0 +1,7 @@
+#include "nm_step_kernel.h"
+
+hipError_t nm_launch_step_lean(int N, hipStream_t s, const nm::Model<float>* M_dev, const nm::Args<float>& a) {
+  constexpr int G = NM_ENVS_PER_WAVE, W = kWG;
+  hipLaunchKernelGGL((k_env_step<float, G, 0, nm::CfgLean>), dim3((N + G * W - 1) / (G * W)), dim3(64 * W), 0, s, M_dev, a);
+  return hipGetLastError();
+}
diff --git a/nightmare_rl_amd/csrc/simt.h b/nightmare_rl_amd/csrc/simt.h
--- a/nightmare_rl_amd/csrc/simt.h
+++ b/nightmare_rl_amd/csrc/simt.h
@@ -58,6 +58,14 @@
 
 NM_FN float vfma(float a, float b, float c) { return __builtin_fmaf(a, b, c); }
 NM_FN double vfma(double a, double b, double c) { return __builtin_fma(a, b, c); }
+NM_FN float vsub_rn(float a, float b) {
+#pragma clang fp contract(off)
+  return a - b;
+}
+NM_FN double vsub_rn(double a, double b) {
+#pragma clang fp contract(off)
+  return a - b;
+}
 NM_FN float sel_mask(uint64_t m, float a, float b) {
   float r;
   asm("v_cndmask_b32_e64 %0, %1, %2, %3" : "=v"(r) : "v"(b), "v"(a), "s"(m));
@@ -272,6 +280,7 @@
 template <class T, class S> NM_FN V<T> vcvt(const V<S>& a) { V<T> r; for (int i = 0; i < NM_WAVE; i++) r.v[i] = (T)a.v[i]; return r; }
 
 template <class T> NM_FN V<T> vfma(const V<T>& a, const V<T>& b, const V<T>& c) { return a * b + c; }
+template <class A, class B> NM_FN auto vsub_rn(const A& a, const B& b) { return a - b; }
 NM_FN float vfma(float a, float b, float c) { return a * b + c; }
 NM_FN double vfma(double a, double b, double c) { return a * b + c; }
 template <class T> NM_FN V<T> sel_mask(uint64_t m, const V<T>& a, const V<T>& b) {
diff --git a/nightmare_rl_amd/envs/nightmare_v3_env.py b/nightmare_rl_amd/envs/nightmare_v3_env.py
--- a/nightmare_rl_amd/envs/nightmare_v3_env.py
+++ b/nightmare_rl_amd/envs/nightmare_v3_env.py
@@ -806,6 +806,12 @@
         self._ret_acc = t
         self._ck(self._L.nm_set_return_accumulator(self._h, None if t is None else t.data_ptr()))
 
+    def set_step_variant(self, generic):
+        self._ck(self._L.nm_set_step_variant(self._h, 1 if generic else 0))
+
+    def step_variant(self):
+        return "lean" if self._L.nm_get_step_variant(self._h) == 1 else "generic"
+
     def profile(self, enable):
         ms, cnt = C.c_double(0), C.c_int64(0)
         self._ck(self._L.nm_profile(self._h, int(bool(enable)), C.byref(ms), C.byref(cnt)))
```

New measurement: 88.31 million env-steps/s (median of 6 runs). 1.02x the previous value.
